# BUTSpeechFIT/DiariZen

Hardware: AMD Instinct MI355X
Metric: audio-seconds/s (RTF) for wavlm-large-s80 pipeline, 16 kHz mono (higher is better)
Workload: dtype f32 (operands split into 2 fp16 terms with exact power-of-two scaling = 22 significant bits, 3 fp16 MFMA products, fp32 accumulate: the error-corrected '3xFP16/3xTF32' scheme; kernels without an fp16 variant use the 3-term bf16 split)

## Files before the change

diarizen_amd/_lib.py:

```python
from __future__ import annotations

import ctypes as C
import os
from pathlib import Path

DZN_MAX_CONV = 8
DZN_MAX_LAYERS = 32
DZN_MAX_HEADS = 16

DZN_PREC_F32 = 0
DZN_PREC_BF16 = 1
DZN_PREC_F32_SPLIT = 2
DZN_PREC_F32_H2 = 3
DZN_PREC_F16 = 4

DZN_ACT_NONE, DZN_ACT_GELU, DZN_ACT_SWISH, DZN_ACT_RELU = 0, 1, 2, 3

DZN_F32, DZN_F64, DZN_I64 = 0, 1, 2

ERRORS = {0: "ok", -1: "invalid argument", -2: "out of memory", -3: "HIP runtime error",
          -4: "bad call order", -5: "missing state_dict key"}


class DznError(RuntimeError):
    pass


class DznConfig(C.Structure):
    _fields_ = [
        ("struct_size", C.c_int32),
        ("precision", C.c_int32),
        ("max_batch", C.c_int32),
        ("max_samples", C.c_int32),
        ("extractor_layer_norm", C.c_int32),
        ("normalize_waveform", C.c_int32),
        ("n_conv", C.c_int32),
        ("conv_ch", C.c_int32 * DZN_MAX_CONV),
        ("conv_k", C.c_int32 * DZN_MAX_CONV),
        ("conv_s", C.c_int32 * DZN_MAX_CONV),
        ("embed_dim", C.c_int32),
        ("total_heads", C.c_int32),
        ("n_layers", C.c_int32),
        ("layer_norm_first", C.c_int32),
        ("pos_conv_kernel", C.c_int32),
        ("pos_conv_groups", C.c_int32),
        ("num_buckets", C.c_int32),
        ("max_distance", C.c_int32),
        ("use_attention", C.c_int32 * DZN_MAX_LAYERS),
        ("n_heads", C.c_int32 * DZN_MAX_LAYERS),
        ("head_idx", (C.c_int32 * DZN_MAX_HEADS) * DZN_MAX_LAYERS),
        ("use_ffn", C.c_int32 * DZN_MAX_LAYERS),
        ("ffn_dim", C.c_int32 * DZN_MAX_LAYERS),
        ("attention_in", C.c_int32),
        ("ffn_hidden", C.c_int32),
        ("conf_heads", C.c_int32),
        ("conf_layers", C.c_int32),
        ("conf_kernel", C.c_int32),
        ("n_classes", C.c_int32),
        ("max_speakers_per_chunk", C.c_int32),
        ("max_speakers_per_frame", C.c_int32),
        ("has_embedding", C.c_int32),
        ("embed_out_dim", C.c_int32),
        ("num_mel_bins", C.c_int32),
        ("reserved", C.c_int32 * 16),
    ]


class DznGemmDesc(C.Structure):
    _fields_ = [
        ("A", C.c_void_p), ("W", C.c_void_p), ("W16", C.c_void_p), ("C", C.c_void_p),
        ("bias", C.c_void_p), ("R", C.c_void_p), ("WS", C.c_void_p),
        ("a_rowoff", C.c_void_p), ("c_rowoff", C.c_void_p),
        ("M", C.c_int32), ("N", C.c_int32), ("K", C.c_int32),
        ("lda", C.c_int64), ("kc", C.c_int32), ("ldk", C.c_int64), ("ldw", C.c_int32),
        ("ldc", C.c_int64), ("ldws", C.c_int64),
        ("act", C.c_int32), ("alpha", C.c_float), ("post_relu", C.c_int32),
        ("ws_w", C.c_float), ("ws_init", C.c_int32),
        ("nz", C.c_int32), ("zdiv", C.c_int32),
        ("a_z0", C.c_int64), ("a_z1", C.c_int64), ("w_z0", C.c_int64), ("w_z1", C.c_int64),
        ("c_z0", C.c_int64), ("c_z1", C.c_int64), ("b_z0", C.c_int64), ("b_z1", C.c_int64),
        ("precision", C.c_int32),
        ("alg_flops", C.c_double),
        ("a_bf16", C.c_int32), ("c_bf16", C.c_int32), ("r_bf16", C.c_int32),
        ("W3", C.c_void_p),
        ("a_split3", C.c_int32), ("a_plane", C.c_int64),
        ("ln_stats", C.c_void_p), ("ln_colsum", C.c_void_p),
        ("W2h", C.c_void_p), ("col_scale", C.c_void_p), ("a_amax", C.c_void_p), ("c_amax", C.c_void_p),
        ("amax_unit", C.c_int32),
        ("stat_partial", C.c_void_p), ("stat_final", C.c_void_p), ("stat_C", C.c_int32), ("stat_eps", C.c_float),
        ("z_count", C.c_void_p), ("z_list", C.c_void_p), ("ln_centered", C.c_int32),
        ("Wmx", C.c_void_p), ("col_scale_mx", C.c_void_p),
        ("amax_count", C.c_int32),
        ("kv_planes", C.c_void_p), ("kv_plane_stride", C.c_int64), ("kv_scale", C.c_void_p), ("kv_ld", C.c_int32),
        ("kv_col0", C.c_int32),
    ]


class DznProfEntry(C.Structure):
    _fields_ = [("name", C.c_char * 64), ("launches", C.c_int64), ("ms", C.c_double),
                ("flops", C.c_double), ("bytes", C.c_double)]


def lib_path() -> Path:
    env = os.environ.get("DZN_HIP_LIB")
    if env:
        return Path(env)
    return Path(__file__).resolve().parent / "lib" / "libdzn_hip.so"


_LIB = None


def load() -> C.CDLL:
    global _LIB
    if _LIB is not None:
        return _LIB
    p = lib_path()
    if not p.exists():
        raise DznError(
            f"{p} not found: build the HIP extension first (python -m diarizen_amd.build). "
            "diarizen_amd has no CPU fallback.")
    try:
        import torch
    except Exception:
        pass
    lib = C.CDLL(str(p))
    vp, i32, i64, f32 = C.c_void_p, C.c_int32, C.c_int64, C.c_float

    def sig(name, res, args):
        fn = getattr(lib, name)
        fn.restype = res
        fn.argtypes = args

    sig("dzn_create", i32, [C.POINTER(DznConfig), C.POINTER(vp)])
    sig("dzn_load_tensor", i32, [vp, C.c_char_p, vp, C.POINTER(i64), i32, i32])
    sig("dzn_finalize_weights", i32, [vp])
    sig("dzn_num_frames", i32, [vp, i32])
    sig("dzn_segment_forward", i32, [vp, vp, i32, i32, vp, vp, vp])
    sig("dzn_embed_forward", i32, [vp, vp, vp, i32, i32, i32, i32, vp, vp])
    sig("dzn_prepare_masks", i32, [vp, vp, i32, i32, i32, i32, i32, vp, vp, vp])
    sig("dzn_speaker_count", i32, [vp, i32, i32, i32, vp, i32, vp, vp, vp])
    sig("dzn_cluster_activations", i32, [vp, vp, i32, i32, i32, vp, i32, i32, vp, vp])
    sig("dzn_detect", i32, [vp, i32, i32, i32, vp, vp, i32, i32, f32, f32, vp, vp, vp])
    sig("dzn_debug_fetch", i32, [vp, C.c_char_p, vp, i64, C.POINTER(i64)])
    sig("dzn_embed_skip_stats", i32, [vp, C.POINTER(i64), C.POINTER(i64)])
    sig("dzn_num_ignored", i32, [vp])
    sig("dzn_workspace_bytes", i64, [vp])
    sig("dzn_last_error", C.c_char_p, [vp])
    sig("dzn_destroy", i32, [vp])
    sig("dzn_version", C.c_char_p, [])
    sig("dzn_profile_enable", i32, [i32])
    sig("dzn_profile_collect", i32, [C.POINTER(DznProfEntry), i32, C.POINTER(i32)])
    sig("dzn_profile_reserve", i32, [i32])
    sig("dzn_op_relpos_bucket", i32, [i32, i32, i32])
    sig("dzn_linkage_centroid", i32, [vp, i32, i32, vp, i32])
    sig("dzn_cdist_cosine", i32, [vp, i32, i32, vp, i32, vp, i32])
    sig("dzn_host_workspace_release", i32, [i32])
    sig("dzn_host_workspace_bytes", i64, [i32])
    sig("dzn_vbx_create", i32, [vp, vp, vp, i32, i32, i32, i32, C.POINTER(C.c_void_p)])
    sig("dzn_vbx_stats", i32, [vp, vp])
    sig("dzn_vbx_estep", i32, [vp, vp, vp, vp, C.c_double, C.POINTER(C.c_double)])
    sig("dzn_vbx_gamma", i32, [vp, vp])
    sig("dzn_vbx_destroy", i32, [vp])
    sig("dzn_op_gemm", i32, [C.POINTER(DznGemmDesc), vp])
    sig("dzn_op_split_weights", i32, [vp, i64, i32, i64, vp, vp])
    sig("dzn_op_split_weights_h2", i32, [vp, i64, i32, i64, vp, vp, vp])
    sig("dzn_op_split_weights_mx", i32, [vp, i64, i32, i64, vp, vp, vp])
    sig("dzn_op_set_gemm_mx_cfg", i32, [C.c_char_p])
    sig("dzn_checked_status", i32, [vp, i32])
    sig("dzn_flac_info", i32, [vp, C.c_size_t, vp, vp, vp, vp, vp])
    sig("dzn_flac_decode", i32, [vp, C.c_size_t, vp, i64, vp])
    sig("dzn_op_set_gemm_cfg", i32, [C.c_char_p])
    sig("dzn_op_amax", i32, [vp, i64, vp, vp])
    sig("dzn_op_split_rows", i32, [vp, vp, i64, i64, i32, vp])
    sig("dzn_op_conv3x3_c32", i32, [vp, vp, vp, vp, vp, i32, i32, i32, i32, i32, vp])
    sig("dzn_op_resblock_ws", i32, [vp, vp, vp, vp, vp, vp, vp, vp, vp, f32, f32, i32, i32, i32, i32, vp])
    sig("dzn_op_resblock32_fused", i32, [vp, vp, vp, vp, vp, vp, vp, vp, vp, f32, f32, i32, i32, i32, vp])
    sig("dzn_op_set_resblock_np", i32, [i32])
    sig("dzn_op_set_attention_noskip", i32, [i32])
    sig("dzn_op_conv3x3_c32_h2", i32, [vp, vp, vp, vp, vp, vp, vp, vp, i32, i32, i32, i32, i32, vp])
    sig("dzn_op_layernorm", i32, [vp, i64, vp, i64, vp, vp, i64, i32, i32, f32, i32, vp])
    sig("dzn_op_gate", i32, [vp, i64, vp, vp, vp, vp, i64, i32, vp])
    sig("dzn_op_row_stats", i32, [vp, i64, i64, i32, f32, vp, vp])
    sig("dzn_op_gate_stats", i32, [vp, i64, vp, vp, vp, vp, vp, vp, vp, i64, i32, f32, vp])
    sig("dzn_op_attention_h2", i32, [vp, vp, vp, vp, vp, i32, i32, i32, i32, i32, i32, f32, vp, vp])
    sig("dzn_op_set_attention_qb", i32, [i32])
    sig("dzn_op_set_attention_prefetch", i32, [i32])
    sig("dzn_op_attention_planes", i32, [vp, vp, vp, vp, vp, i32, i32, i32, i32, i32, i32, f32, vp, vp, vp, vp])
    sig("dzn_op_attention", i32, [vp, vp, vp, vp, vp, i32, i32, i32, i32, i32, i32, f32, i32, vp])
    _LIB = lib
    return lib


EXPORTED = [
    "dzn_create", "dzn_load_tensor", "dzn_finalize_weights", "dzn_num_frames",
    "dzn_segment_forward", "dzn_embed_forward", "dzn_prepare_masks", "dzn_speaker_count", "dzn_cluster_activations", "dzn_detect", "dzn_debug_fetch", "dzn_embed_skip_stats", "dzn_num_ignored",
    "dzn_workspace_bytes", "dzn_last_error", "dzn_destroy", "dzn_version", "dzn_linkage_centroid", "dzn_cdist_cosine", "dzn_host_workspace_release",
    "dzn_host_workspace_bytes",
    "dzn_flac_info", "dzn_flac_decode", "dzn_vbx_create", "dzn_vbx_stats", "dzn_vbx_estep", "dzn_vbx_gamma", "dzn_vbx_destroy",
    "dzn_op_gemm", "dzn_op_split_weights", "dzn_op_split_weights_h2", "dzn_op_split_weights_mx", "dzn_op_set_gemm_mx_cfg", "dzn_checked_status", "dzn_op_set_gemm_cfg", "dzn_op_amax", "dzn_op_conv3x3_c32", "dzn_op_conv3x3_c32_h2", "dzn_op_resblock32_fused", "dzn_op_resblock_ws", "dzn_op_set_resblock_np", "dzn_op_set_attention_noskip", "dzn_op_split_rows", "dzn_op_layernorm", "dzn_op_row_stats", "dzn_op_gate", "dzn_op_gate_stats", "dzn_op_attention", "dzn_op_attention_h2", "dzn_op_attention_planes", "dzn_op_set_attention_qb", "dzn_op_set_attention_prefetch",
    "dzn_profile_enable", "dzn_profile_collect", "dzn_profile_reserve", "dzn_op_relpos_bucket",
]


def profile_enable(on: bool) -> None:
    check(load().dzn_profile_enable(int(on)), None, "dzn_profile_enable")


def profile_reserve(n_events: int) -> None:
    check(load().dzn_profile_reserve(int(n_events)), None, "dzn_profile_reserve")


def profile_collect() -> list:
    lib = load()
    arr = (DznProfEntry * 512)()
    n = C.c_int32(0)
    check(lib.dzn_profile_collect(arr, 512, C.byref(n)), None, "dzn_profile_collect")
    return [dict(name=arr[i].name.decode(), launches=arr[i].launches, ms=arr[i].ms,
                 flops=arr[i].flops, bytes=arr[i].bytes) for i in range(min(n.value, 512))]


def check(rc: int, handle=None, what: str = "") -> None:
    if rc == 0:
        return
    msg = ERRORS.get(rc, f"error {rc}")
    try:
        detail = load().dzn_last_error(handle)
        if detail:
            msg += ": " + detail.decode(errors="replace")
    except Exception:
        pass
    if rc == -2:
        raise MemoryError(f"{what}: {msg}")
    raise DznError(f"{what}: {msg}")
```

diarizen_amd/csrc/attention.hip:

```cpp
#include "common.h"

namespace {

template <bool BIAS, typename TO>
__global__ __launch_bounds__(256) void attn_kernel(const float* __restrict__ qkv,
                                                   TO* __restrict__ out,
                                                   const float* __restrict__ gate,
                                                   const float* __restrict__ table,
                                                   const int32_t* __restrict__ head_idx, int B,
                                                   int L, int h, int Htot, int ldqkv, int ldo,
                                                   float scale) {
  extern __shared__ __attribute__((aligned(16))) float smem_f[];
  float* sK = smem_f;
  float* sV = smem_f + 64 * 64;
  float* sT = smem_f + 2 * 64 * 64;

  const int tid = threadIdx.x, lane = tid & 63, wave = tid >> 6;
  const int lr = lane & 15, lq = lane >> 4;
  const int qt = blockIdx.x, j = blockIdx.y, b = blockIdx.z;
  const int64_t rowbase = (int64_t)b * L;
  const float* Qp = qkv + j * 64;
  const float* Kp = qkv + (h + j) * 64;
  const float* Vp = qkv + (2 * h + j) * 64;

// ... 205 lines not shown
  float wa[16], wb[16];
#pragma unroll
  for (int j = 0; j < 16; ++j) {
    wa[j] = sw[sub * 16 + j];
    wb[j] = sw[64 + sub * 16 + j];
  }
  const float ba = sw[128], bb = sw[129];
  const int C = Htot * 64;
  float gm[MAXI], bt[MAXI];
#pragma unroll
  for (int i = 0; i < MAXI; ++i) {
    gm[i] = i < Htot ? gamma[lane + 64 * i] : 0.f;
    bt[i] = i < Htot ? beta[lane + 64 * i] : 0.f;
  }
  float* sr = sy[wave];
  for (int64_t row = (int64_t)blockIdx.x * 4 + wave; row < rows; row += (int64_t)gridDim.x * 4) {
    const float* xp = x + row * ldx;
    float v[MAXI];
    float sum = 0.f;
#pragma unroll
    for (int i = 0; i < MAXI; ++i) {
      v[i] = i < Htot ? xp[lane + 64 * i] : 0.f;
      sum += v[i];
    }
    const float mean = wave_sum(sum) / (float)C;
    float sq = 0.f;
#pragma unroll
    for (int i = 0; i < MAXI; ++i) {
      const float dv = i < Htot ? v[i] - mean : 0.f;
      sq += dv * dv;
    }
    const float rstd = 1.0f / sqrtf(wave_sum(sq) / (float)C + eps);
    if (lane == 0) *reinterpret_cast<float2*>(stats + 2 * row) = make_float2(mean, rstd);
    __builtin_amdgcn_wave_barrier();
#pragma unroll
    for (int i = 0; i < MAXI; ++i)
      if (i < Htot) {
        const int e = lane + 64 * i;
        sr[e + (e >> 4)] = (v[i] - mean) * rstd * gm[i] + bt[i];
      }
    __builtin_amdgcn_s_waitcnt(0xc07f);
    __builtin_amdgcn_wave_barrier();
    for (int H0 = 0; H0 < Htot; H0 += 16) {
      const int H = H0 + (lane >> 2);
      float ta = 0.f, tb = 0.f;
      if (H < Htot) {
        const int e0 = H * 64 + sub * 16;
        const float* yp = sr + e0 + (e0 >> 4);
#pragma unroll
        for (int j = 0; j < 16; ++j) {
          ta = fmaf(yp[j], wa[j], ta);
          tb = fmaf(yp[j], wb[j], tb);
        }
      }
      ta = dpp_add<0xB1, 0xF>(ta);
      ta = dpp_add<0x4E, 0xF>(ta);
      tb = dpp_add<0xB1, 0xF>(tb);
      tb = dpp_add<0x4E, 0xF>(tb);
      if (H < Htot && sub == 0) {
        const float ga = 1.0f / (1.0f + expf(-(ta + ba)));
        const float gb = 1.0f / (1.0f + expf(-(tb + bb)));
        gate[row * Htot + H] = ga * (gb * cst[H] - 1.0f) + 2.0f;
      }
    }
  }
}

}

int launch_gate_stats(const float* x, int64_t ldx, const float* gamma, const float* beta, const float* Wg,
                      const float* bg, const float* cst, float* gate, float* stats, int64_t rows, int Htot, float eps,
                      hipStream_t s) {
  if (rows <= 0) return DZN_OK;
  if (Htot < 1 || Htot > 16) return DZN_E_INVALID;
  int pid = prof_enabled() ? prof_begin(s, "gate_ln_stats", 0.0, (double)rows * Htot * 64 * 4.0) : -1;
  int64_t grid = cdiv64(rows, 4);
  grid = grid > 256 * 8 ? 256 * 8 : grid;
  hipLaunchKernelGGL(gate_stats_kernel<16>, dim3((unsigned)grid), dim3(256), 0, s, x, ldx, gamma, beta, Wg,
                     bg, cst, gate, stats, rows, Htot, eps);
  prof_end(pid, s);
  return hipGetLastError() == hipSuccess ? DZN_OK : DZN_E_HIP;
}

extern "C" int dzn_op_gate_stats(const float* x, int64_t ldx, const float* gamma, const float* beta, const float* Wg,
                                 const float* bg, const float* cst, float* gate, float* stats, int64_t rows,
                                 int32_t Htot, float eps, void* stream) {
  if (!x || !gamma || !beta || !Wg || !bg || !cst || !gate || !stats) return DZN_E_INVALID;
  return launch_gate_stats(x, ldx, gamma, beta, Wg, bg, cst, gate, stats, rows, Htot, eps,
                           reinterpret_cast<hipStream_t>(stream));
}

int launch_attention_t(const float* qkv, void* out, int out_bf16, const float* gate, const float* table,
                       const int32_t* head_idx, int B, int L, int h, int Htot, int ldqkv, int ldo,
                       float scale, hipStream_t s) {
  if (h <= 0 || B <= 0 || L <= 0) return DZN_OK;
  const bool bias = gate && table && head_idx;
  const size_t lds = (2 * 64 * 64 + (bias ? (2 * L - 1) : 0)) * sizeof(float);
  if (lds > 160 * 1024) return DZN_E_INVALID;
  dim3 grid((L + 63) / 64, h, B);
  const int pid = prof_begin(s, bias ? "attention_relpos_f32" : "attention_f32",
                             4.0 * B * h * (double)L * L * 64.0,
                             (double)B * L * h * 64.0 * 4.0 * 4.0 + (gate ? (double)B * L * Htot * 4.0 : 0.0));
#define DZN_ATT(BIASV, T)                                                                          \
  hipLaunchKernelGGL((attn_kernel<BIASV, T>), grid, dim3(256), lds, s, qkv, static_cast<T*>(out), gate, \
                     table, head_idx, B, L, h, Htot, ldqkv, ldo, scale)
  if (bias) {
    if (out_bf16) DZN_ATT(true, u16); else DZN_ATT(true, float);
  } else {
    if (out_bf16) DZN_ATT(false, u16); else DZN_ATT(false, float);
  }
#undef DZN_ATT
  prof_end(pid, s);
  return hipGetLastError() == hipSuccess ? DZN_OK : DZN_E_HIP;
}

int launch_attention(const float* qkv, float* out, const float* gate, const float* table,
                     const int32_t* head_idx, int B, int L, int h, int Htot, int ldqkv, int ldo,
                     float scale, int precision, hipStream_t s) {
  if (prec_is_split(precision))
    return launch_attention_split(qkv, out, gate, table, head_idx, B, L, h, Htot, ldqkv, ldo, scale, s);
  return launch_attention_t(qkv, out, 0, gate, table, head_idx, B, L, h, Htot, ldqkv, ldo, scale, s);
}

int launch_gate_t(const void* y, int y_bf16, int64_t ldy, const float* Wg, const float* bg,
                  const float* cst, float* gate, int64_t rows, int Htot, hipStream_t s) {
  ProfScope prof_scope_(s, "gate", 0.0, (double)rows * Htot * (64.0 + 1.0) * 4.0);
  if (rows <= 0) return DZN_OK;
  if (y_bf16)
    hipLaunchKernelGGL(gate_kernel<u16>, dim3((unsigned)cdiv64(rows, 4)), dim3(256), 0, s,
                       static_cast<const u16*>(y), ldy, Wg, bg, cst, gate, rows, Htot);
  else
    hipLaunchKernelGGL(gate_kernel<float>, dim3((unsigned)cdiv64(rows, 4)), dim3(256), 0, s,
                       static_cast<const float*>(y), ldy, Wg, bg, cst, gate, rows, Htot);
  return hipGetLastError() == hipSuccess ? DZN_OK : DZN_E_HIP;
}

int launch_gate(const float* y, int64_t ldy, const float* Wg, const float* bg, const float* cst,
                float* gate, int64_t rows, int Htot, hipStream_t s) {
  return launch_gate_t(y, 0, ldy, Wg, bg, cst, gate, rows, Htot, s);
}

extern "C" int dzn_op_attention(const float* qkv, float* out, const float* gate,
                                const float* table, const int32_t* head_idx, int32_t B, int32_t L,
                                int32_t h, int32_t Htot, int32_t ldqkv, int32_t ldo, float scale,
                                int32_t precision, void* stream) {
  if (!qkv || !out) return DZN_E_INVALID;
  return launch_attention(qkv, out, gate, table, head_idx, B, L, h, Htot, ldqkv, ldo, scale,
                          precision, reinterpret_cast<hipStream_t>(stream));
}

extern "C" int dzn_op_gate(const float* y, int64_t ldy, const float* Wg, const float* bg,
                           const float* cst, float* gate, int64_t rows, int32_t Htot,
                           void* stream) {
  return launch_gate(y, ldy, Wg, bg, cst, gate, rows, Htot, reinterpret_cast<hipStream_t>(stream));
}
```

diarizen_amd/csrc/common.h:

```cpp
#pragma once
#include <hip/hip_runtime.h>
#include <stdint.h>
#include <math.h>
#include <string.h>
#include "../../include/dzn.h"
#include "../../include/dzn_ops.h"

typedef float f32x4 __attribute__((ext_vector_type(4)));
typedef __bf16 bf16x8 __attribute__((ext_vector_type(8)));
typedef __bf16 bf16x4 __attribute__((ext_vector_type(4)));
typedef unsigned short u16;

#define DZN_WAVE 64

template <int CTRL, int ROW_MASK>
__device__ __forceinline__ float dpp_add(float v) {
  const int t = __builtin_amdgcn_update_dpp(ROW_MASK == 0xF ? __float_as_int(v) : 0, __float_as_int(v), CTRL,
                                            ROW_MASK, 0xF, false);
  return v + __int_as_float(t);
}
__device__ __forceinline__ float wave_sum(float v) {
  v = dpp_add<0xB1, 0xF>(v);
  v = dpp_add<0x4E, 0xF>(v);
  v = dpp_add<0x124, 0xF>(v);
// ... 6 lines not shown
#pragma unroll
  for (int o = 32; o > 0; o >>= 1) v = fmaxf(v, __shfl_xor(v, o, 64));
  return v;
}

__device__ __forceinline__ void track_amax_lane(float* tracker, float m) {
  if (m > 0.f) {
    const unsigned cur = __hip_atomic_load(reinterpret_cast<unsigned int*>(tracker), __ATOMIC_RELAXED, __HIP_MEMORY_SCOPE_AGENT);
    if (__float_as_uint(m) > cur) atomicMax(reinterpret_cast<unsigned int*>(tracker), __float_as_uint(m));
  }
}
__device__ __forceinline__ void track_amax(float* tracker, float wave_partial) {
  const float m = wave_max(wave_partial);
  if ((threadIdx.x & 63) == 0) track_amax_lane(tracker, m);
}

__device__ __forceinline__ float erf_as(float x) {
  const float ax = fabsf(x);
  const float t = __builtin_amdgcn_rcpf(fmaf(0.3275911f, ax, 1.0f));
  float p = fmaf(1.061405429f, t, -1.453152027f);
  p = fmaf(p, t, 1.421413741f);
  p = fmaf(p, t, -0.284496736f);
  p = fmaf(p, t, 0.254829592f);
  const float e = __builtin_amdgcn_exp2f(-1.4426950408889634f * ax * ax);
  const float y = fmaf(-p * t, e, 1.0f);
  return copysignf(y, x);
}
__device__ __forceinline__ float gelu_erf(float x) {
  return 0.5f * x * (1.0f + erf_as(x * 0.70710678118654752440f));
}
__device__ __forceinline__ float sigmoidf_(float x) { return 1.0f / (1.0f + expf(-x)); }
__device__ __forceinline__ float swishf_(float x) { return x * sigmoidf_(x); }

__device__ __forceinline__ float apply_act(float v, int act) {
  switch (act) {
    case DZN_ACT_GELU: return gelu_erf(v);
    case DZN_ACT_SWISH: return swishf_(v);
    case DZN_ACT_RELU: return fmaxf(v, 0.0f);
    default: return v;
  }
}

__device__ __forceinline__ float ld_act(const float* p, int64_t i) { return p[i]; }
__device__ __forceinline__ float ld_act(const u16* p, int64_t i) {
  return __uint_as_float(((unsigned int)p[i]) << 16);
}
__device__ __forceinline__ void st_act(float* p, int64_t i, float v) { p[i] = v; }
__device__ __forceinline__ void st_act(u16* p, int64_t i, float v) {
  __bf16 h = (__bf16)v;
  p[i] = *reinterpret_cast<u16*>(&h);
}

static inline u16 f32_to_bf16_host(float f) {
  uint32_t u;
  memcpy(&u, &f, 4);
  if ((u & 0x7fffffffu) > 0x7f800000u) return (u16)((u >> 16) | 0x40);
  uint32_t r = 0x7fffu + ((u >> 16) & 1u);
  return (u16)((u + r) >> 16);
}

static inline bool prec_is_h2(int p) { return p == DZN_PREC_F32_H2 || p == DZN_PREC_F16; }
static inline bool prec_is_split(int p) { return p == DZN_PREC_F32_SPLIT || prec_is_h2(p); }

int launch_gemm(const dzn_gemm_desc& d, hipStream_t s);
#ifdef DZN_TUNING
int launch_gemm_lowp(const dzn_gemm_desc& d, hipStream_t s);
#endif
int launch_gemm_split(const dzn_gemm_desc& d, hipStream_t s);
int launch_gemm_split_pre(const dzn_gemm_desc& d, hipStream_t s);
int launch_pad_rows_split3(const float* x, void* planes, int64_t plane_stride, int B, int L, int Lp, int pad, int D,
                           hipStream_t st, int cg = 0, int cgp = 0);
int launch_pad_rows_split2(const float* x, void* planes, int64_t plane_stride, int B, int L, int Lp, int pad, int D,
                           const float* amax, float* snapshot, hipStream_t st, int cg = 0, int cgp = 0);
int launch_split_weights(const float* W, int64_t rows, int K, int64_t ldw, void* W3, hipStream_t s);
int launch_split_weights_h2(const float* W, int64_t rows, int K, int64_t ldw, void* W2, float* col_scale, hipStream_t s);
int host_stage_stream(int device, hipStream_t* stream);
int host_state_lease(int device, size_t bytes, hipStream_t* stream, char** base);
void host_state_release(int device);
int launch_gemm_mx(const dzn_gemm_desc& d, hipStream_t s);
int launch_split_weights_mx(const float* W, int64_t rows, int K, int64_t ldw, void* Wmx, float* col_scale, hipStream_t s);
int launch_amax(const float* x, int64_t n, float* amax, hipStream_t s);
int launch_fill_u32(void* p, unsigned value, int64_t n, hipStream_t st);
int launch_stats_finalize(const float* partial, int64_t rows, int P, int C, float eps, float* stats, hipStream_t s);
int launch_layernorm(const float* x, int64_t ldx, float* y, int64_t ldy, const float* g,
                     const float* b, int64_t rows, int C, int Cpad, float eps, int gelu,
                     hipStream_t s);
int launch_layernorm_t(const void* x, int x_bf16, int64_t ldx, void* y, int y_bf16, int64_t ldy,
                       const float* g, const float* b, const float* post, int64_t rows, int C, int Cpad,
                       float eps, int gelu, hipStream_t s, float* amax = nullptr, int64_t amax_unit = 0);
int launch_cast_bf16(const float* x, void* y, int64_t n, hipStream_t s);
int launch_row_stats(const float* x, int64_t ldx, int64_t rows, int C, float eps, float* stats, hipStream_t s);
int launch_gate_stats(const float* x, int64_t ldx, const float* gamma, const float* beta, const float* Wg,
                      const float* bg, const float* cst, float* gate, float* stats, int64_t rows, int Htot, float eps,
                      hipStream_t s);
int launch_wave_stats(const float* w, int B, int N, float eps, float* stats, hipStream_t s);
int launch_gate(const float* y, int64_t ldy, const float* Wg, const float* bg, const float* cst,
                float* gate, int64_t rows, int Htot, hipStream_t s);
int launch_gate_t(const void* y, int y_bf16, int64_t ldy, const float* Wg, const float* bg,
                  const float* cst, float* gate, int64_t rows, int Htot, hipStream_t s);
int launch_attention_t(const float* qkv, void* out, int out_bf16, const float* gate, const float* table,
                       const int32_t* head_idx, int B, int L, int h, int Htot, int ldqkv, int ldo,
                       float scale, hipStream_t s);
int launch_attention_split(const float* qkv, float* out, const float* gate, const float* table,
                           const int32_t* head_idx, int B, int L, int h, int Htot, int ldqkv, int ldo,
                           float scale, hipStream_t s, const float* amax = nullptr);
int launch_attention(const float* qkv, float* out, const float* gate, const float* table,
                     const int32_t* head_idx, int B, int L, int h, int Htot, int ldqkv, int ldo,
                     float scale, int precision, hipStream_t s);
int launch_attention_planes(const float* qkv, const void* planes, int64_t plane_stride, const float* kvs, int kv_ld, float* out,
                            const float* gate, const float* table, const int32_t* head_idx, int B, int L, int h, int Htot,
                            int ldqkv, int ldo, float scale, hipStream_t s, const float* amax);

int launch_conv0(const float* wave, int B, int N, const float* stats, const float* w,
                 const float* gamma, const float* beta, int C0, int Cp, int k, int s, int T0,
                 int layer_norm, float eps, void* out, int out_bf16, hipStream_t st, const float* lnq = nullptr);
int launch_groupnorm_gelu(const float* x, void* y, int y_bf16, int B, int T, int C, int Cp, int64_t ld,
                          const float* gamma, const float* beta, float eps, float* stats, hipStream_t st, float* amax = nullptr);
int64_t gn_stats_floats(int B, int T, int C, int Cp);
int launch_pad_rows(const float* x, void* xpad, int out_bf16, int B, int L, int Lp, int pad, int D,
                    hipStream_t st);
int launch_ws_accum(const float* x, float* ws, float w, int init, int64_t n, hipStream_t st);
constexpr int WS_SUM_MAX = 40;
struct WsSumArgs {
  const float* x[WS_SUM_MAX];
  float w[WS_SUM_MAX];
  int n;
};
int launch_ws_sum(const WsSumArgs& a, float* ws, int64_t n, hipStream_t st);
int launch_col_scale(void* x, int x_bf16, int64_t rows, int C, int64_t ld, const float* scale,
                     hipStream_t st);
int launch_split_weights_h2_natural(const float* W, int64_t rows, int K, void* W2, float* col_scale, hipStream_t s);
int launch_fragment_major(const void* W2, int rows, int K, void* out, hipStream_t s);
int launch_conv01_fused(const float* wave, int B, int N, const float* wstats, const float* w0, const float* gamma0,
                        const float* beta0, const float* lnq, int C0, int T0, int T1, const void* W2h,
                        const float* col_scale, int N1p, float act_bound, float eps, float* out, hipStream_t st,
                        const float* gamma1 = nullptr, const float* beta1 = nullptr, int C1 = 0, float* amax1 = nullptr);
int launch_glu_dwconv(const float* u, int64_t ldu, const float* w, const float* bias, void* out,
                      int out_bf16, int64_t ldo, int B, int L, int A, int ks, hipStream_t st);
int launch_classify(const float* z, int64_t ldz, const float* W, const float* bias,
                    const uint8_t* mapping, int64_t rows, int A, int NC, int S, float* logp,
                    uint8_t* multilabel, hipStream_t st);
int launch_frame_prep(const float* wave, int B, int N, int T, int flen, int fshift, int Kp,
                      const float* window, float preemph, float* frames, hipStream_t st);
int launch_power(const float* spec, int64_t rows, int nb, float* pw, hipStream_t st);
int launch_window_active(const float* masks, int B, int per_window, int* flag, hipStream_t st);
int launch_compact_active(const int* flag, int B, int* count, int* list, long long* totals, hipStream_t st);
int launch_log_cmn(float* mel, int B, int T, int NB, float eps, hipStream_t st);
int launch_stem_conv(const float* fb, int B, int T, int NB, int C, const float* w, const float* bias,
                     void* img, int out_bf16, hipStream_t st, float* amax = nullptr, const int* z_count = nullptr,
                     const int* z_list = nullptr);
int launch_stats_pool(const void* img, int in_bf16, int B, int H, int W, int C, const float* masks, int S,
                      int L, float* stats, hipStream_t st, const int* active = nullptr);

int launch_conv3x3_c32_split(const float* in, const void* W3, const float* bias, const float* R, float* out, int B,
                             int Hs, int Ws, int relu, int post_relu, hipStream_t s, float* amax = nullptr,
                             const void* W2h = nullptr, const float* col_scale = nullptr, const float* amax_in = nullptr,
                             const int* z_count = nullptr, const int* z_list = nullptr);

int launch_resblock32_fused(const float* in, float* out, const void* W1, const float* cs1, const float* b1, const void* W2,
                            const float* cs2, const float* b2, const float* amax_in, float* amax_out, float l1max1,
                            float bmax1, int B, int Hs, int Ws, int np, hipStream_t s, const int* z_count = nullptr,
                            const int* z_list = nullptr);

int launch_resblock_ws(const float* in, float* out, const void* W1, const float* cs1, const float* b1, const void* W2,
                       const float* cs2, const float* b2, const float* amax_in, float* amax_out, float l1max1, float bmax1,
                       int B, int Hs, int Ws, int C, hipStream_t s, const int* z_count = nullptr, const int* z_list = nullptr,
// ... 60 lines not shown
```

diarizen_amd/csrc/engine.cpp:

```cpp
#include <algorithm>
#include <cmath>
#include <cstdio>
#include <cstdlib>
#include <map>
#include <set>
#include <stdexcept>
#include <string>
#include <vector>

#include "common.h"

#define HIPCHK(x)                                                                        \
  do {                                                                                   \
    hipError_t e_ = (x);                                                                 \
    if (e_ != hipSuccess) {                                                              \
      throw EngineError(e_ == hipErrorOutOfMemory ? DZN_E_NOMEM : DZN_E_HIP,             \
                        std::string(#x) + ": " + hipGetErrorString(e_));                 \
    }                                                                                    \
  } while (0)

namespace {

struct EngineError : std::runtime_error {
  int code;
  EngineError(int c, const std::string& m) : std::runtime_error(m), code(c) {}
};


struct HostT {
  std::vector<float> v;
  std::vector<int64_t> shape;
};

struct Lin {
  float* W = nullptr;
  u16* W16 = nullptr;
  u16* W3 = nullptr;
  float* b = nullptr;
  u16* W2h = nullptr;
  float* wsc = nullptr;
  float* csum = nullptr;
  unsigned char* Wmx = nullptr;
  float* wsc_mx = nullptr;
  int N = 0, K = 0;
  int Nt = 0, Kt = 0;
};

struct LNp {
  float* g = nullptr;
  float* b = nullptr;
  int C = 0;
};

struct EncLayer {
  bool attn = false, ffn = false;
  int h = 0, F = 0, Fp = 0;
  LNp ln1, ln2;
  Lin qkv, out, f1, f2;
  float *Wg = nullptr, *bg = nullptr, *cst = nullptr;
  int32_t* head_idx = nullptr;
};

struct ConfLayer {
  LNp ffn1_ln, ffn2_ln, mha_ln, conv_ln, out_ln;
  Lin ffn1_w1, ffn1_w2, ffn2_w1, ffn2_w2, qkv, o, pw1, pw2;
  float *dw = nullptr, *dwb = nullptr;
};

struct ResConv {
  Lin l;
  int cin = 0, cout = 0, ksz = 3, stride = 1;
  float l1max = 0.f, bmax = 0.f;
};
struct ResBlock {
  ResConv c1, c2, sc;
  bool has_sc = false;
};

std::string last_create_error;

const char* const F16_CLASSES[] = {"conv gemm", "feature projection", "pos conv", "qkv", "out_proj", "ffn1", "ffn2", "proj",
                                   "conf ffn w1", "conf ffn w2", "conf qkv", "conf out", "conf pw1", "conf pw2"};
int f16_class(const char* what) {
  for (int i = 0; i < (int)(sizeof(F16_CLASSES) / sizeof(F16_CLASSES[0])); ++i)
    if (!strcmp(what, F16_CLASSES[i])) return i;
  return -1;
}

}

struct dzn_handle {
  dzn_config cfg{};
  int device = 0;
  std::string err;
  std::map<std::string, HostT> sd;
  std::set<std::string> used;
  int ignored = 0;
  bool finalized = false;
  bool debug = false;
  std::vector<void*> allocs;
  int64_t bytes = 0;
  std::map<std::string, std::vector<float>> taps;

  int nconv = 0;
  int C[DZN_MAX_CONV]{}, Cp[DZN_MAX_CONV]{};
  int D = 0, H = 0, A = 0, Fh = 0;
  float* conv0_w = nullptr;
  float* conv0_lnq = nullptr;
  u16* conv1_W2n = nullptr;
  float* conv1_wscn = nullptr;
  LNp conv_ln[DZN_MAX_CONV];
  Lin conv[DZN_MAX_CONV];
  float* dummy_w = nullptr;
  LNp fp_ln, enc_ln;
  Lin fp, posconv;
  int pos_rowD = 0;
  int pos_cgp = 0;
  std::vector<EncLayer> layers;
  std::vector<float> rel_embed;
  std::vector<float> wsum_w;
  Lin proj;
  LNp lnorm;
  std::vector<ConfLayer> conf;
  float *cls_w = nullptr, *cls_b = nullptr;
  uint8_t* mapping = nullptr;
  int table_L = -1;
  int pos_L = -1;
  int32_t* pos_rowoff = nullptr;
  u16* xpad3 = nullptr;
  int64_t xpad3_plane = 0;
  float* table = nullptr;
  int maxT[DZN_MAX_CONV]{};
  int maxL = 0;
  float *stats = nullptr, *gn_stats = nullptr, *bufA = nullptr, *bufB = nullptr, *craw = nullptr;
  float *x = nullptr, *xpad = nullptr, *y = nullptr, *ws = nullptr, *qkv = nullptr, *ao = nullptr,
        *gate = nullptr, *mid = nullptr;
  float *hz = nullptr, *ht = nullptr, *hmid = nullptr, *hv = nullptr;
  void* kvp = nullptr;
  float* kvs = nullptr;
  int64_t kvp_rows = 0;
  int kvp_ldmax = 0;
  float* xl = nullptr;
// ... 318 lines not shown
    }
  }
  const int last = c.n_conv - 1;
  {
    const HostT& dw = need(h, P + "feature_extractor.dummy_weight");
    expect_numel(dw, h->C[last], "dummy_weight");
    h->dummy_w = upload(h, dw.v);
  }
  const int D = h->D;
  h->fp_ln = ln_from_sd(h, P + "encoder.feature_projection.layer_norm", h->C[last]);
  if (h->fold_ln)
    h->fp = linear_ln_from_sd(h, P + "encoder.feature_projection.projection",
                              P + "encoder.feature_projection.layer_norm", D, h->C[last], D, h->Cp[last]);
  else
    h->fp = linear_from_sd(h, P + "encoder.feature_projection.projection", D, h->C[last], D,
                           h->Cp[last]);
  {
    const std::string pc = P + "encoder.transformer.pos_conv_embed.conv";
    const HostT& g = need(h, pc + ".parametrizations.weight.original0");
    const HostT& v = need(h, pc + ".parametrizations.weight.original1");
    const HostT& b = need(h, pc + ".bias");
    const int K = c.pos_conv_kernel, G = c.pos_conv_groups, cg = D / G;
    expect_numel(g, K, pc + ".original0");
    expect_numel(v, (int64_t)D * cg * K, pc + ".original1");
    expect_numel(b, D, pc + ".bias");
    std::vector<double> nrm(K, 0.0);
    for (int o = 0; o < D; ++o)
      for (int ii = 0; ii < cg; ++ii)
        for (int j = 0; j < K; ++j) {
          const double t = v.v[((size_t)o * cg + ii) * K + j];
          nrm[j] += t * t;
        }
    const int cgp = prec_is_split(c.precision) ? round_up(cg, 32) : cg;
    h->pos_cgp = cgp;
    std::vector<float> wp((size_t)D * K * cgp, 0.f);
    for (int o = 0; o < D; ++o)
      for (int ii = 0; ii < cg; ++ii)
        for (int j = 0; j < K; ++j) {
          const float nj = (float)std::sqrt(nrm[j]);
          wp[((size_t)o * K + j) * cgp + ii] = g.v[j] * v.v[((size_t)o * cg + ii) * K + j] / nj;
        }
    h->posconv = make_lin(h, wp, b.v.data(), D, K * cgp, D, K * cgp);
    h->posconv.Kt = K * cg;
  }
  if (!c.layer_norm_first) h->enc_ln = ln_from_sd(h, P + "encoder.transformer.layer_norm", D);
  h->layers.resize(c.n_layers);
  int maxQ = 64, maxF = 32;
  for (int i = 0; i < c.n_layers; ++i) {
    EncLayer& L = h->layers[i];
    const std::string lp = P + "encoder.transformer.layers." + std::to_string(i);
    L.attn = c.use_attention[i] && c.n_heads[i] > 0;
    L.ffn = c.use_ffn[i] != 0;
    L.ln1 = ln_from_sd(h, lp + ".layer_norm", D);
    L.ln2 = ln_from_sd(h, lp + ".final_layer_norm", D);
    if (L.attn) {
      L.h = c.n_heads[i];
      const int hd = L.h * 64;
      maxQ = std::max(maxQ, hd);
      std::vector<float> wq((size_t)3 * hd * D), bq((size_t)3 * hd);
      const char* names[3] = {".attention.q_proj", ".attention.k_proj", ".attention.v_proj"};
      for (int t = 0; t < 3; ++t) {
        const HostT& w = need(h, lp + names[t] + ".weight");
        const HostT& b = need(h, lp + names[t] + ".bias");
        expect_numel(w, (int64_t)hd * D, lp + names[t] + ".weight");
        expect_numel(b, hd, lp + names[t] + ".bias");
        std::copy(w.v.begin(), w.v.end(), wq.begin() + (size_t)t * hd * D);
        std::copy(b.v.begin(), b.v.end(), bq.begin() + (size_t)t * hd);
      }
      if (h->fold_ln && c.layer_norm_first)
        L.qkv = make_lin_ln(h, wq, bq.data(), need(h, lp + ".layer_norm.weight").v,
                            need(h, lp + ".layer_norm.bias").v, 3 * hd, D, 3 * hd, D);
      else
        L.qkv = make_lin(h, wq, bq.data(), 3 * hd, D, 3 * hd, D);
      L.out = linear_from_sd(h, lp + ".attention.out_proj", D, hd, D, hd);
      const HostT& wg = need(h, lp + ".attention.gru_rel_pos_linear.weight");
      const HostT& bg = need(h, lp + ".attention.gru_rel_pos_linear.bias");
      const HostT& cs = need(h, lp + ".attention.gru_rel_pos_const");
      expect_numel(wg, 8 * 64, "gru_rel_pos_linear.weight");
      expect_numel(bg, 8, "gru_rel_pos_linear.bias");
      expect_numel(cs, h->H, "gru_rel_pos_const");
      L.Wg = upload(h, wg.v);
      L.bg = upload(h, bg.v);
      L.cst = upload(h, cs.v);
      std::vector<int32_t> hi(c.head_idx[i], c.head_idx[i] + L.h);
      for (int v : hi)
        if (v < 0 || v >= h->H) throw EngineError(DZN_E_INVALID, "head index out of range");
      L.head_idx = dalloc<int32_t>(h, L.h, false);
      HIPCHK(hipMemcpy(L.head_idx, hi.data(), L.h * sizeof(int32_t), hipMemcpyHostToDevice));
      if (i == 0) {
        const HostT& e = need(h, lp + ".attention.rel_attn_embed.weight");
        expect_numel(e, (int64_t)c.num_buckets * h->H, "rel_attn_embed.weight");
        h->rel_embed = e.v;
      }
    }
    if (L.ffn) {
      L.F = c.ffn_dim[i];
      L.Fp = pad32(L.F);
      maxF = std::max(maxF, L.Fp);
      if (h->fold_ln && c.layer_norm_first)
        L.f1 = linear_ln_from_sd(h, lp + ".feed_forward.intermediate_dense", lp + ".final_layer_norm", L.F, D,
                                 L.Fp, D);
      else
        L.f1 = linear_from_sd(h, lp + ".feed_forward.intermediate_dense", L.F, D, L.Fp, D);
      L.f2 = linear_from_sd(h, lp + ".feed_forward.output_dense", D, L.F, D, L.Fp);
    }
  }
  if (h->rel_embed.empty())
    throw EngineError(DZN_E_INVALID, "layer 0 must carry attention (rel_attn_embed lives there)");
  {
    const HostT& w = need(h, "weight_sum.weight");
    expect_numel(w, c.n_layers + 1, "weight_sum.weight");
    h->wsum_w = w.v;
  }
  const int A = h->A, Fh = h->Fh;
  h->proj = linear_from_sd(h, "proj", A, D, A, D);
  h->lnorm = ln_from_sd(h, "lnorm", A);
  h->conf.resize(c.conf_layers);
  for (int i = 0; i < c.conf_layers; ++i) {
    ConfLayer& L = h->conf[i];
    const std::string cp = "conformer.conformer_layer." + std::to_string(i);
    L.ffn1_ln = ln_from_sd(h, cp + ".ffn1.ln_norm", A);
    L.ffn1_w1 = h->fold_ln ? linear_ln_from_sd(h, cp + ".ffn1.w_1", cp + ".ffn1.ln_norm", Fh, A, Fh, A)
                           : linear_from_sd(h, cp + ".ffn1.w_1", Fh, A, Fh, A);
    L.ffn1_w2 = linear_from_sd(h, cp + ".ffn1.w_2", A, Fh, A, Fh);
    L.ffn2_ln = ln_from_sd(h, cp + ".ffn2.ln_norm", A);
    L.ffn2_w1 = h->fold_ln ? linear_ln_from_sd(h, cp + ".ffn2.w_1", cp + ".ffn2.ln_norm", Fh, A, Fh, A)
                           : linear_from_sd(h, cp + ".ffn2.w_1", Fh, A, Fh, A);
    L.ffn2_w2 = linear_from_sd(h, cp + ".ffn2.w_2", A, Fh, A, Fh);
    L.mha_ln = ln_from_sd(h, cp + ".mha.ln_norm", A);
    {
      std::vector<float> wq((size_t)3 * A * A), bq((size_t)3 * A);
      const char* names[3] = {".mha.mha.linearQ", ".mha.mha.linearK", ".mha.mha.linearV"};
      for (int t = 0; t < 3; ++t) {
        const HostT& w = need(h, cp + names[t] + ".weight");
        const HostT& b = need(h, cp + names[t] + ".bias");
        expect_numel(w, (int64_t)A * A, cp + names[t] + ".weight");
        expect_numel(b, A, cp + names[t] + ".bias");
        std::copy(w.v.begin(), w.v.end(), wq.begin() + (size_t)t * A * A);
        std::copy(b.v.begin(), b.v.end(), bq.begin() + (size_t)t * A);
      }
      if (h->fold_ln)
        L.qkv = make_lin_ln(h, wq, bq.data(), need(h, cp + ".mha.ln_norm.weight").v,
                            need(h, cp + ".mha.ln_norm.bias").v, 3 * A, A, 3 * A, A);
      else
        L.qkv = make_lin(h, wq, bq.data(), 3 * A, A, 3 * A, A);
    }
    L.o = linear_from_sd(h, cp + ".mha.mha.linearO", A, A, A, A);
    L.conv_ln = ln_from_sd(h, cp + ".conv.ln_norm", A);
    L.pw1 = h->fold_ln ? linear_ln_from_sd(h, cp + ".conv.pointwise_conv1", cp + ".conv.ln_norm", 2 * A, A, 2 * A, A)
                       : linear_from_sd(h, cp + ".conv.pointwise_conv1", 2 * A, A, 2 * A, A);
    L.pw2 = linear_from_sd(h, cp + ".conv.pointwise_conv2", A, A, A, A);
    {
      const int ks = c.conf_kernel;
      const HostT& w = need(h, cp + ".conv.depthwise_conv.weight");
      const HostT& b = need(h, cp + ".conv.depthwise_conv.bias");
      const HostT& g = need(h, cp + ".conv.bn_norm.weight");
      const HostT& be = need(h, cp + ".conv.bn_norm.bias");
      const HostT& rm = need(h, cp + ".conv.bn_norm.running_mean");
      const HostT& rv = need(h, cp + ".conv.bn_norm.running_var");
      expect_numel(w, (int64_t)A * ks, cp + ".conv.depthwise_conv.weight");
      std::vector<float> wf((size_t)A * ks), bf(A);
      for (int ch = 0; ch < A; ++ch) {
        const float s = g.v[ch] / std::sqrt(rv.v[ch] + 1e-5f);
        for (int j = 0; j < ks; ++j) wf[(size_t)ch * ks + j] = w.v[(size_t)ch * ks + j] * s;
        bf[ch] = (b.v[ch] - rm.v[ch]) * s + be.v[ch];
      }
// ... 467 lines not shown
  const bool fold = h->fold_ln;
  auto folded = [&](dzn_gemm_desc& d, const Lin& l) {
    d.ln_stats = h->rstat;
    d.ln_colsum = l.csum;
  };
  if (fold) {
    chk(launch_row_stats(cur, h->Cp[last], ML, h->C[last], 1e-5f, h->rstat, st), "row_stats");
    dzn_gemm_desc d = gd(h, cur, h->fp, h->x, ML, h->Cp[last], D);
    folded(d, h->fp);
    if (lnx && c.n_conv > 1) d.a_amax = am(conv_slot(cur));
    d.c_amax = am(dzn_handle::AM_X);
    gemm(d, false, false, "feature projection");
  } else {
    ln_t(cur, lp, h->Cp[last], nxt, lp, h->Cp[last], h->fp_ln, ML, h->Cp[last], 0, st);
    dzn_gemm_desc d = gd(h, nxt, h->fp, h->x, ML, h->Cp[last], D);
    d.c_amax = am(dzn_handle::AM_X);
    gemm(d, lp, false, "feature projection");
  }
  tap(h, "featproj", h->x, ML, D, D, st);

  {
    const int Kc = c.pos_conv_kernel, G = c.pos_conv_groups, cg = D / G, Lp = L + Kc;
    const bool pc16 = lp && (cg % 32 == 0);
    const int cgp = h->pos_cgp > 0 ? h->pos_cgp : cg, Dp = G * cgp;
    const bool pre3 = h->xpad3 != nullptr && (int64_t)c.max_batch * Lp * Dp < (int64_t)1 << 31;
    const bool pre2 = pre3 && h2 && h->posconv.W2h;
    if (pre2)
      chk(launch_pad_rows_split2(h->x, h->xpad3, h->xpad3_plane, B, L, Lp, Kc / 2, Dp, am(dzn_handle::AM_X),
                                 am(dzn_handle::AM_XPAD), st, cg, cgp),
          "pad_rows_split2");
    else if (pre3)
      chk(launch_pad_rows_split3(h->x, h->xpad3, h->xpad3_plane, B, L, Lp, Kc / 2, Dp, st, cg, cgp), "pad_rows_split3");
    else
      chk(launch_pad_rows(h->x, h->xpad, pc16, B, L, Lp, Kc / 2, D, st), "pad_rows");
    const int ca = pre3 ? cgp : cg, Da = pre3 ? Dp : D;
    if (!pre3 && cgp != cg) throw EngineError(DZN_E_INVALID, "padded positional-conv groups need the pre-split planes");
    const bool tabled = (int64_t)c.max_batch * Lp * Da < (int64_t)1 << 31;
    if (tabled) ensure_pos_rowoff(h, L, Lp, Da, st);
    dzn_gemm_desc d = gd(h, h->xpad, h->posconv, h->x, tabled ? ML : L, Da, D);
    d.N = cg;
    d.kc = ca;
    d.ldk = Da;
    d.act = DZN_ACT_GELU;
    d.R = h->x;
    d.a_z1 = ca;
    d.w_z1 = (int64_t)cg * h->posconv.K;
    d.c_z1 = cg;
    d.b_z1 = cg;
    if (tabled) {
      d.a_rowoff = h->pos_rowoff;
      d.nz = G;
      d.zdiv = G;
      d.alg_flops = 2.0 * (double)ML * cg * h->posconv.Kt;
    } else {
      d.nz = B * G;
      d.zdiv = G;
      d.a_z0 = (int64_t)Lp * Da;
      d.c_z0 = (int64_t)L * D;
      d.alg_flops = 2.0 * (double)L * cg * h->posconv.Kt;
    }
    if (pre3) {
      d.A = reinterpret_cast<const float*>(h->xpad3);
      d.a_split3 = pre2 ? 2 : 1;
      d.a_plane = h->xpad3_plane;
      if (pre2) d.a_amax = am(dzn_handle::AM_XPAD);
    }
    d.c_amax = am(dzn_handle::AM_X);
    gemm(d, pc16, false, "pos conv");
  }
  if (!c.layer_norm_first) ln_t(h->x, false, D, h->x, false, D, h->enc_ln, ML, D, 0, st, nullptr, am(dzn_handle::AM_X), L);
  const bool defer = h->xl != nullptr;
  float* xr = h->x;
  WsSumArgs wsum{};
  if (defer) {
    wsum.x[wsum.n] = xr;
    wsum.w[wsum.n++] = h->wsum_w[0];
  } else {
    chk(launch_ws_accum(h->x, h->ws, h->wsum_w[0], 1, ML * D, st), "ws_accum");
  }
  tap(h, "rep0", h->x, ML, D, D, st);

  static const bool stats_from_epilogue = getenv("DZN_NO_EPILOGUE_STATS") == nullptr;
  ensure_table(h, L, st);
  for (int i = 0; i < c.n_layers; ++i) {
    EncLayer& Ly = h->layers[i];
    const float wl = h->wsum_w[i + 1];
    float* const own = defer ? h->xl + (int64_t)i * ML * D : xr;
    bool have_stats = false;
    if (Ly.attn) {
      const float* yin = xr;
      bool y16 = false;
      const bool fold1 = fold && c.layer_norm_first;
      if (fold1) {
        chk(launch_gate_stats(xr, D, Ly.ln1.g, Ly.ln1.b, Ly.Wg, Ly.bg, Ly.cst, h->gate, h->rstat, ML, h->H, 1e-5f,
                              st),
            "gate_stats");
      } else if (c.layer_norm_first) {
        ln_t(xr, false, D, h->y, lp, D, Ly.ln1, ML, D, 0, st, nullptr, am(dzn_handle::AM_Y), L);
        yin = h->y;
        y16 = lp;
      } else if (lp) {
        chk(launch_cast_bf16(xr, h->y, ML * D, st), "cast");
        yin = h->y;
        y16 = true;
      }
      if (!fold1) chk(launch_gate_t(yin, y16, D, Ly.Wg, Ly.bg, Ly.cst, h->gate, ML, h->H, st), "gate");
      const int hd = Ly.h * 64;
      dzn_gemm_desc d = gd(h, yin, Ly.qkv, h->qkv, ML, D, 3 * hd);
      if (fold1) folded(d, Ly.qkv);
      d.a_amax = am(yin == xr ? dzn_handle::AM_X : dzn_handle::AM_Y);
      d.c_amax = am(dzn_handle::AM_QKV);
      const bool planes = h->kvp != nullptr && !y16 && d.W2h && d.col_scale && d.a_amax;
      const int64_t pstride = (ML + 64) * (int64_t)(2 * hd);
      if (planes) {
        d.kv_planes = h->kvp;
        d.kv_plane_stride = pstride;
        d.kv_scale = h->kvs;
        d.kv_ld = 2 * hd;
        d.kv_col0 = hd;
      }
      gemm(d, y16, false, "qkv");
      if (planes)
        chk(launch_attention_planes(h->qkv, h->kvp, pstride, h->kvs, 2 * hd, h->ao, h->gate, h->table, Ly.head_idx, B, L, Ly.h, h->H,
                                    3 * hd, hd, 0.125f, st, am(dzn_handle::AM_QKV)),
            "attention");
      else if (prec_is_split(c.precision))
        chk(launch_attention_split(h->qkv, h->ao, h->gate, h->table, Ly.head_idx, B, L, Ly.h, h->H, 3 * hd, hd,
                                   0.125f, st, am(dzn_handle::AM_QKV)),
            "attention");
      else
        chk(launch_attention_t(h->qkv, h->ao, lp, h->gate, h->table, Ly.head_idx, B, L, Ly.h, h->H, 3 * hd,
                               hd, 0.125f, st),
            "attention");
      dzn_gemm_desc o = gd(h, h->ao, Ly.out, own, ML, hd, D);
      o.R = xr;
      o.a_amax = am(dzn_handle::AM_QKV);
      o.c_amax = am(dzn_handle::AM_X);
      if (fold && c.layer_norm_first && Ly.ffn && stats_from_epilogue) {
        o.stat_partial = h->spart;
        o.stat_final = h->rstat;
        o.stat_C = D;
        o.stat_eps = 1e-5f;
        have_stats = true;
      }
      gemm(o, lp, false, "out_proj");
      xr = own;
    }
    if (c.layer_norm_first) {
      if (Ly.ffn) {
        const float* fin = h->y;
        if (fold) {
          if (!have_stats) chk(launch_row_stats(xr, D, ML, D, 1e-5f, h->rstat, st), "row_stats");
          fin = xr;
        } else {
          ln_t(xr, false, D, h->y, lp, D, Ly.ln2, ML, D, 0, st, nullptr, am(dzn_handle::AM_Y), L);
        }
        dzn_gemm_desc f1 = gd(h, fin, Ly.f1, h->mid, ML, D, Ly.Fp);
        if (fold) folded(f1, Ly.f1);
        f1.act = DZN_ACT_GELU;
        f1.a_amax = am(fin == xr ? dzn_handle::AM_X : dzn_handle::AM_Y);
        f1.c_amax = am(dzn_handle::AM_MID);
        gemm(f1, lp, lp, "ffn1");
        dzn_gemm_desc f2 = gd(h, h->mid, Ly.f2, own, ML, Ly.Fp, D);
        f2.R = xr;
        if (!defer) {
          f2.WS = h->ws;
          f2.ldws = D;
          f2.ws_w = wl;
        }
        f2.a_amax = am(dzn_handle::AM_MID);
        f2.c_amax = am(dzn_handle::AM_X);
        gemm(f2, lp, false, "ffn2");
        xr = own;
      } else if (!defer) {
        chk(launch_ws_accum(xr, h->ws, wl, 0, ML * D, st), "ws_accum");
      }
      if (defer) {
        wsum.x[wsum.n] = xr;
        wsum.w[wsum.n++] = wl;
      }
    } else {
      ln_t(xr, false, D, xr, false, D, Ly.ln1, ML, D, 0, st, nullptr, am(dzn_handle::AM_X), L);
      if (Ly.ffn) {
        const float* fin = xr;
        if (lp) {
          chk(launch_cast_bf16(xr, h->y, ML * D, st), "cast");
          fin = h->y;
        }
        dzn_gemm_desc f1 = gd(h, fin, Ly.f1, h->mid, ML, D, Ly.Fp);
        f1.act = DZN_ACT_GELU;
        f1.a_amax = am(dzn_handle::AM_X);
        f1.c_amax = am(dzn_handle::AM_MID);
        gemm(f1, lp, lp, "ffn1");
        dzn_gemm_desc f2 = gd(h, h->mid, Ly.f2, xr, ML, Ly.Fp, D);
        f2.R = xr;
        f2.a_amax = am(dzn_handle::AM_MID);
        f2.c_amax = am(dzn_handle::AM_X);
        gemm(f2, lp, false, "ffn2");
      }
      ln_t(xr, false, D, xr, false, D, Ly.ln2, ML, D, 0, st, nullptr, am(dzn_handle::AM_X), L);
      chk(launch_ws_accum(xr, h->ws, wl, 0, ML * D, st), "ws_accum");
    }
    if (h->debug) {
      const std::string nm = "layer" + std::to_string(i);
      tap(h, nm.c_str(), xr, ML, D, D, st);
    }
  }
  if (defer) chk(launch_ws_sum(wsum, h->ws, ML * D, st), "ws_sum");
  tap(h, "wsum", h->ws, ML, D, D, st);

  {
    const float* pin = h->ws;
    if (lp) {
      chk(launch_cast_bf16(h->ws, h->y, ML * D, st), "cast");
      pin = h->y;
    }
    dzn_gemm_desc d = gd(h, pin, h->proj, h->hz, ML, D, A);
    gemm(d, lp, false, "proj");
    ln_t(h->hz, false, A, h->hz, false, A, h->lnorm, ML, A, 0, st, nullptr, am(dzn_handle::AM_HZ), L);
  }
  tap(h, "head_in", h->hz, ML, A, A, st);
  for (int i = 0; i < c.conf_layers; ++i) {
    ConfLayer& Cl = h->conf[i];
    auto half_ffn = [&](const LNp& ln, const Lin& w1, const Lin& w2) {
      const float* in = h->ht;
      if (fold) {
        chk(launch_row_stats(h->hz, A, ML, A, 1e-5f, h->rstat, st), "row_stats");
        in = h->hz;
      } else {
        ln_t(h->hz, false, A, h->ht, lp, A, ln, ML, A, 0, st);
      }
      dzn_gemm_desc a = gd(h, in, w1, h->hmid, ML, A, Fh);
      if (fold) folded(a, w1);
      a.act = DZN_ACT_SWISH;
      if (in == h->hz) a.a_amax = am(dzn_handle::AM_HZ);
      a.c_amax = am(dzn_handle::AM_HMID);
      gemm(a, lp, lp, "conf ffn w1");
      dzn_gemm_desc b = gd(h, h->hmid, w2, h->hz, ML, Fh, A);
      b.alpha = 0.5f;
      b.R = h->hz;
      b.a_amax = am(dzn_handle::AM_HMID);
      b.c_amax = am(dzn_handle::AM_HZ);
      gemm(b, lp, false, "conf ffn w2");
    };
    half_ffn(Cl.ffn1_ln, Cl.ffn1_w1, Cl.ffn1_w2);
    if (fold) chk(launch_row_stats(h->hz, A, ML, A, 1e-5f, h->rstat, st), "row_stats");
    else ln_t(h->hz, false, A, h->ht, lp, A, Cl.mha_ln, ML, A, 0, st);
    {
      dzn_gemm_desc q = gd(h, fold ? h->hz : h->ht, Cl.qkv, h->hmid, ML, A, 3 * A);
      if (fold) {
        folded(q, Cl.qkv);
        q.a_amax = am(dzn_handle::AM_HZ);
      }
      q.c_amax = am(dzn_handle::AM_HMID);
// ... 477 lines not shown
```

diarizen_amd/csrc/gemm.hip:

```cpp
#include <cstdio>
#include <cstdlib>

#include "common.h"
#include "gemm_epilogue.h"

namespace {

template <bool LOWP>
struct Frag {
  using type = f32x4;
};
template <>
struct Frag<true> {
  using type = bf16x8;
};

__device__ __forceinline__ uint4 pack_bf16x8(const float4& a, const float4& b) {
  bf16x8 v;
  v[0] = (__bf16)a.x; v[1] = (__bf16)a.y; v[2] = (__bf16)a.z; v[3] = (__bf16)a.w;
  v[4] = (__bf16)b.x; v[5] = (__bf16)b.y; v[6] = (__bf16)b.z; v[7] = (__bf16)b.w;
  return *reinterpret_cast<uint4*>(&v);
}

template <int BM, int BN, int WGM, int WGN, bool LOWP>
// ... 284 lines not shown
    __syncthreads();
    if (more) read_frags(buf ^ 1, 0, a0, b0);
    __builtin_amdgcn_sched_barrier(0);
    mma(a1, b1);
    __builtin_amdgcn_sched_barrier(0);
  }
  gemm_epilogue<BM, BN, TM, TN, MI, NI>(d, acc, tm, tn, wm, wn, lr, lq, cz, bz, z0);
}

template <int BM, int BN, int WGM, int WGN, bool LOWP>
int launch_cfg(const dzn_gemm_desc& d, hipStream_t s) {
  const int tilesM = (d.M + BM - 1) / BM, tilesN = (d.N + BN - 1) / BN;
  static const int lds_pad = getenv("DZN_GEMM_LDS_PAD") ? atoi(getenv("DZN_GEMM_LDS_PAD")) : 0;
  const size_t lds = 2 * (BM + BN) * 128 + lds_pad;
  auto kern = gemm_kernel<BM, BN, WGM, WGN, LOWP>;
  static unsigned long long attr_mask = 0;
  if (first_use_on_device(attr_mask)) {
    (void)hipFuncSetAttribute(reinterpret_cast<const void*>(kern),
                        hipFuncAttributeMaxDynamicSharedMemorySize, 160 * 1024);
    if constexpr (!LOWP)
      (void)hipFuncSetAttribute(reinterpret_cast<const void*>(gemm_glds_kernel<BM, BN, WGM, WGN>),
                                hipFuncAttributeMaxDynamicSharedMemorySize, 160 * 1024);
  }
  static const bool no_glds = getenv("DZN_NO_GLDS") != nullptr;
  const bool use_glds = !LOWP && !no_glds && (d.K % 32 == 0) && (d.kc % 32 == 0);
  dim3 grid(tilesM * tilesN, d.nz > 0 ? d.nz : 1, 1);
  int pid = -1;
  if (prof_enabled()) {
    char cls[64];
    static const bool by_shape = getenv("DZN_PROFILE_SHAPES") != nullptr;
    if (by_shape)
      snprintf(cls, sizeof(cls), "gemm_%s_%dx%d M%d N%d K%d z%d", LOWP ? "bf16" : "f32", BM, BN, d.M, d.N,
               d.K, d.nz);
    else
      snprintf(cls, sizeof(cls), "gemm_%s_%dx%d", LOWP ? "bf16" : "f32", BM, BN);
    const double fl = d.alg_flops > 0 ? d.alg_flops * d.nz : 2.0 * d.M * d.N * d.K * d.nz;
    pid = prof_begin(s, cls, fl, gemm_alg_bytes(d, LOWP ? 2 : 4));
  }
  if constexpr (!LOWP) {
    if (use_glds)
      hipLaunchKernelGGL((gemm_glds_kernel<BM, BN, WGM, WGN>), grid, dim3(256), lds, s, d);
    else
      hipLaunchKernelGGL(kern, grid, dim3(256), lds, s, d);
  } else {
    hipLaunchKernelGGL(kern, grid, dim3(256), lds, s, d);
  }
  prof_end(pid, s);
  if (hipGetLastError() != hipSuccess) return DZN_E_HIP;
  if (d.stat_partial && d.stat_final)
    return launch_stats_finalize(d.stat_partial, d.M, ((d.N + BN - 1) / BN) * WGN, d.stat_C, d.stat_eps, d.stat_final, s);
  return DZN_OK;
}

template <bool LOWP>
int launch_prec(const dzn_gemm_desc& d, hipStream_t s) {
  static const char* force = getenv("DZN_GEMM_CFG");
  if (force) {
    if (!strcmp(force, "128x32")) return launch_cfg<128, 32, 4, 1, LOWP>(d, s);
    if (!strcmp(force, "256x32")) return launch_cfg<256, 32, 4, 1, LOWP>(d, s);
    if (!strcmp(force, "256x64")) return launch_cfg<256, 64, 4, 1, LOWP>(d, s);
    if (!strcmp(force, "128x64")) return launch_cfg<128, 64, 2, 2, LOWP>(d, s);
    if (!strcmp(force, "64x64")) return launch_cfg<64, 64, 2, 2, LOWP>(d, s);
    if (!strcmp(force, "128x128")) return launch_cfg<128, 128, 2, 2, LOWP>(d, s);
  }
  if (d.N <= 32) return launch_cfg<256, 32, 4, 1, LOWP>(d, s);
  if (d.N <= 64) return launch_cfg<128, 64, 2, 2, LOWP>(d, s);
  if (d.K <= 512 && (d.N % 64) == 0) return launch_cfg<128, 64, 2, 2, LOWP>(d, s);
  const int cand[4] = {192, 160, 128, 96};
  int best = 128, best_cols = 1 << 30;
  for (int c : cand) {
    const int cols = (d.N + c - 1) / c * c;
    if (cols < best_cols) { best_cols = cols; best = c; }
  }
  switch (best) {
    case 192: return launch_cfg<128, 192, 2, 2, LOWP>(d, s);
    case 160: return launch_cfg<128, 160, 2, 2, LOWP>(d, s);
    case 96: return launch_cfg<128, 96, 2, 2, LOWP>(d, s);
    default: return launch_cfg<128, 128, 2, 2, LOWP>(d, s);
  }
}

}

int launch_gemm(const dzn_gemm_desc& din, hipStream_t s) {
  dzn_gemm_desc d = din;
  if (d.M <= 0 || d.N <= 0) return DZN_OK;
  if (d.K <= 0 || (d.K & 7)) return DZN_E_INVALID;
  if (d.kc <= 0) { d.kc = d.K; d.ldk = 0; }
  if (d.kc & 7) return DZN_E_INVALID;
  if (d.zdiv <= 0) d.zdiv = 1;
  if (d.nz <= 0) d.nz = 1;
  if (d.alpha == 0.f) d.alpha = 1.f;
  if (d.precision == DZN_PREC_BF16) {
    if (!d.W16) return DZN_E_INVALID;
#ifdef DZN_TUNING
    if (d.a_bf16) return launch_gemm_lowp(d, s);
#else
    if (d.a_bf16) return DZN_E_INVALID;
#endif
    if (d.c_bf16 || d.r_bf16) return DZN_E_INVALID;
    return launch_prec<true>(d, s);
  }
  if (!d.W) return DZN_E_INVALID;
  if (d.kv_planes) {
    const bool ok = d.kv_scale && d.precision == DZN_PREC_F32_H2 && d.W3 && d.W2h && d.col_scale && d.a_amax && !(d.K & 31) &&
                    !(d.kc & 31) && d.ldw == d.K && !d.a_split3 && d.nz == 1 && !d.c_rowoff && d.kv_col0 >= 0 &&
                    d.kv_col0 < d.N && !(d.kv_col0 & 63) && !(d.N & 63) && d.kv_ld == d.N - d.kv_col0 &&
                    !(d.kv_plane_stride & 3) && d.N > 32 && !getenv("DZN_GEMM_CFG") && !getenv("DZN_NO_H2");
    if (!ok) return DZN_E_INVALID;
  }
  if (d.ln_centered && !(d.precision == DZN_PREC_F16 && d.W3 && !(d.K & 31) && !(d.kc & 31) && d.ldw == d.K && !d.a_split3))
    return DZN_E_INVALID;
  if (d.a_split3) return prec_is_split(d.precision) ? launch_gemm_split_pre(d, s) : DZN_E_INVALID;
  if (prec_is_split(d.precision) && d.W3 && !(d.K & 31) && !(d.kc & 31) && d.ldw == d.K)
    return launch_gemm_split(d, s);
  return launch_prec<false>(d, s);
}

extern "C" int dzn_op_gemm(const dzn_gemm_desc* d, void* stream) {
  if (!d || !d->A || !d->C) return DZN_E_INVALID;
  return launch_gemm(*d, reinterpret_cast<hipStream_t>(stream));
}
```

diarizen_amd/csrc/gemm_epilogue.h:

```cpp
#pragma once
#include <type_traits>

#include "common.h"
#include "split.h"

namespace {

template <int BM, int BN, int TM, int TN, int MI, int NI, int RS = 16, int CS = 16>
__device__ __forceinline__ void gemm_epilogue_general(const dzn_gemm_desc& d, f32x4 (&acc)[MI][NI], int tm, int tn,
                                              int wm, int wn, int lr, int lq, int64_t cz, int64_t bz, int z0 = 0,
                                              const float* row_inv = nullptr, const float* col_scale = nullptr) {
  const float* __restrict__ bias = d.bias ? d.bias + bz : nullptr;
  const bool vec = (((int64_t)d.N | d.ldc | d.ldws | cz | bz) & 3) == 0;
  float amax = 0.f, amax_hi = 0.f;
  const int wrow0 = tm * BM + wm * TM;
  const bool two_unit = d.c_amax && d.amax_unit >= TM;
  const int unit0 = two_unit ? (wrow0 < d.M ? wrow0 : d.M - 1) / d.amax_unit : 0;
  const int boundary = two_unit ? (unit0 + 1) * d.amax_unit : 0;
#pragma unroll
  for (int i = 0; i < MI; ++i) {
    const int m = tm * BM + wm * TM + i * RS + lr;
    if (m >= d.M) continue;
    const int64_t crow = cz + (d.c_rowoff ? (int64_t)d.c_rowoff[m] : (int64_t)m * d.ldc);
    const float acc_scale = row_inv ? row_inv[i] : 1.f;
// ... 37 lines not shown
        *reinterpret_cast<float4*>(d.C + crow + n0) = make_float4(v[0], v[1], v[2], v[3]);
        amax_row = fmaxf(fmaxf(amax_row, fmaxf(fabsf(v[0]), fabsf(v[1]))), fmaxf(fabsf(v[2]), fabsf(v[3])));
        st_s += (v[0] + v[1]) + (v[2] + v[3]);
        st_q = fmaf(v[0], v[0], fmaf(v[1], v[1], fmaf(v[2], v[2], fmaf(v[3], v[3], st_q))));
        if (d.WS) {
          float4* w = reinterpret_cast<float4*>(d.WS + (int64_t)m * d.ldws + n0);
          float4 a = d.ws_init ? make_float4(0.f, 0.f, 0.f, 0.f) : *w;
          a.x += d.ws_w * v[0]; a.y += d.ws_w * v[1]; a.z += d.ws_w * v[2]; a.w += d.ws_w * v[3];
          *w = a;
        }
      } else {
#pragma unroll
        for (int e = 0; e < 4; ++e) {
          const int n = n0 + e;
          if (n >= d.N) continue;
          float x = v[e];
          if (col_scale) x *= acc_scale * col_scale[n];
          if (d.ln_stats) x = ln_rs * (x - ln_mu * d.ln_colsum[n]);
          if (bias) x += bias[n];
          x = apply_act(x, d.act) * d.alpha;
          if (d.R) x += d.R[crow + n];
          if (d.post_relu) x = fmaxf(x, 0.f);
          d.C[crow + n] = x;
          amax_row = fmaxf(amax_row, fabsf(x));
          st_s += x;
          st_q = fmaf(x, x, st_q);
          if (d.WS) {
            float* w = d.WS + (int64_t)m * d.ldws + n;
            *w = d.ws_init ? d.ws_w * x : (*w + d.ws_w * x);
          }
        }
      }
    }
    if (d.stat_partial) {
      float s1 = st_s, q1 = st_q;
      if constexpr (RS == 16) {
        s1 += __shfl_xor(s1, 16, 64);
        q1 += __shfl_xor(q1, 16, 64);
      }
      s1 += __shfl_xor(s1, 32, 64);
      q1 += __shfl_xor(q1, 32, 64);
      if (lq == 0) {
        const int P = ((d.N + BN - 1) / BN) * (BN / TN);
        reinterpret_cast<float2*>(d.stat_partial)[(int64_t)m * P + tn * (BN / TN) + wn] = make_float2(s1, q1);
      }
    }
    if (d.c_amax) {
      if (two_unit) {
        if (m < boundary) amax = fmaxf(amax, amax_row);
        else amax_hi = fmaxf(amax_hi, amax_row);
      } else if (d.amax_unit > 0) {
        float r = amax_row;
        if constexpr (RS == 16) r = fmaxf(r, __shfl_xor(r, 16, 64));
        r = fmaxf(r, __shfl_xor(r, 32, 64));
        if (lq == 0) track_amax_lane(d.c_amax + m / d.amax_unit, r);
      } else {
        amax = fmaxf(amax, amax_row);
      }
    }
  }
  if (two_unit) {
    track_amax(d.c_amax + unit0, amax);
    if (wrow0 + TM > boundary && boundary < d.M) track_amax(d.c_amax + unit0 + 1, amax_hi);
  } else if (d.c_amax && d.amax_unit <= 0) {
    track_amax(d.c_amax + z0, amax);
  }
}

constexpr int epi_chunk(int ni, int cap) {
  int best = 1;
  for (int c = 1; c <= cap; ++c)
    if (ni % c == 0) best = c;
  return best;
}

template <int ACT>
__device__ __forceinline__ float apply_act_c(float v) {
  if constexpr (ACT == DZN_ACT_GELU) return gelu_erf(v);
  else if constexpr (ACT == DZN_ACT_SWISH) return swishf_(v);
  else if constexpr (ACT == DZN_ACT_RELU) return fmaxf(v, 0.0f);
  else return v;
}

template <int BM, int BN, int TM, int TN, int MI, int NI, bool LDSCOLS = false, int RS = 16, int CS = 16>
__device__ __forceinline__ void gemm_epilogue(const dzn_gemm_desc& d, f32x4 (&acc)[MI][NI], int tm, int tn,
                                              int wm, int wn, int lr, int lq, int64_t cz, int64_t bz, int z0 = 0,
                                              const float* row_inv = nullptr, const float* col_scale = nullptr,
                                              float* lds_cols = nullptr, const f32x4 (*rpre)[NI] = nullptr) {
  const bool vec = (((int64_t)d.N | d.ldc | d.ldws | cz | bz) & 3) == 0 && d.N >= 4;
  if (!vec) {
    gemm_epilogue_general<BM, BN, TM, TN, MI, NI, RS, CS>(d, acc, tm, tn, wm, wn, lr, lq, cz, bz, z0, row_inv, col_scale);
    return;
  }
  const bool ring = d.R && !rpre;
  constexpr int JCMAX = MI * NI > 16 ? 4 : 8;
  constexpr int JC = epi_chunk(NI, JCMAX);
  static_assert(NI % JC == 0, "column chunks tile the wavefront tile");
  constexpr int NJC = NI / JC, NB = MI * NJC;
  constexpr bool REGCOLS = !LDSCOLS && NI <= 4;
  const float* __restrict__ bias = d.bias ? d.bias + bz : nullptr;
  const int ncol0 = tn * BN + wn * TN + lq * 4;
  auto nok_ = [&](const int j) { return ncol0 + j * CS < d.N; };
  auto nc_ = [&](const int j) {
    const int n0 = ncol0 + j * CS;
    return n0 < d.N ? n0 : d.N - 4;
  };
  int64_t crow[MI];
  bool mok[MI];
  int mcl[MI];
#pragma unroll
  for (int i = 0; i < MI; ++i) {
    const int m = tm * BM + wm * TM + i * RS + lr;
    mok[i] = m < d.M;
    mcl[i] = mok[i] ? m : d.M - 1;
    crow[i] = cz + (d.c_rowoff ? (int64_t)d.c_rowoff[mcl[i]] : (int64_t)mcl[i] * d.ldc);
  }
  float4 r4[2][JC];
  auto issue_r = [&](const int b, const int slot) {
    const int i = b / NJC, jc = b % NJC;
#pragma unroll
    for (int jj = 0; jj < JC; ++jj) r4[slot][jj] = *reinterpret_cast<const float4*>(d.R + crow[i] + nc_(jc * JC + jj));
  };
  if (ring) issue_r(0, 0);
  float ln_mu[MI], ln_rs[MI];
#pragma unroll
  for (int i = 0; i < MI; ++i) {
    ln_mu[i] = 0.f;
    ln_rs[i] = 1.f;
  }
  if (d.ln_stats) {
#pragma unroll
    for (int i = 0; i < MI; ++i) {
      const float2 st = *reinterpret_cast<const float2*>(d.ln_stats + 2 * (int64_t)mcl[i]);
      ln_mu[i] = d.ln_centered ? 0.f : st.x;
      ln_rs[i] = st.y;
    }
  }
  float4 cs4[REGCOLS ? NI : 1], lc4[REGCOLS ? NI : 1], b4[REGCOLS ? NI : 1];
  if constexpr (REGCOLS) {
#pragma unroll
    for (int j = 0; j < NI; ++j) {
      cs4[j] = make_float4(1.f, 1.f, 1.f, 1.f);
      lc4[j] = b4[j] = make_float4(0.f, 0.f, 0.f, 0.f);
    }
    if (col_scale) {
#pragma unroll
      for (int j = 0; j < NI; ++j) cs4[j] = *reinterpret_cast<const float4*>(col_scale + nc_(j));
    }
    if (d.ln_stats) {
#pragma unroll
      for (int j = 0; j < NI; ++j) lc4[j] = *reinterpret_cast<const float4*>(d.ln_colsum + nc_(j));
    }
    if (bias) {
#pragma unroll
      for (int j = 0; j < NI; ++j) b4[j] = *reinterpret_cast<const float4*>(bias + nc_(j));
    }
  } else if constexpr (LDSCOLS) {
    const int lane = lq * RS + lr;
    if (lane < TN / 4) {
      int n = tn * BN + wn * TN + 4 * lane;
      n = n < d.N ? n : d.N - 4;
      float4 c = make_float4(1.f, 1.f, 1.f, 1.f), l = make_float4(0.f, 0.f, 0.f, 0.f), bb = l;
      if (col_scale) c = *reinterpret_cast<const float4*>(col_scale + n);
      if (d.ln_stats) l = *reinterpret_cast<const float4*>(d.ln_colsum + n);
      if (bias) bb = *reinterpret_cast<const float4*>(bias + n);
      *reinterpret_cast<float4*>(lds_cols + 4 * lane) = c;
      *reinterpret_cast<float4*>(lds_cols + TN + 4 * lane) = l;
      *reinterpret_cast<float4*>(lds_cols + 2 * TN + 4 * lane) = bb;
    }
    __builtin_amdgcn_fence(__ATOMIC_RELEASE, "wavefront");
  }
  auto cols = [&](const int j, float4& c, float4& l, float4& bb) {
    if constexpr (REGCOLS) {
      c = cs4[j]; l = lc4[j]; bb = b4[j];
    } else if constexpr (LDSCOLS) {
      const float* p = lds_cols + j * CS + lq * 4;
      c = *reinterpret_cast<const float4*>(p);
      l = *reinterpret_cast<const float4*>(p + TN);
      bb = *reinterpret_cast<const float4*>(p + 2 * TN);
    } else {
      c = col_scale ? *reinterpret_cast<const float4*>(col_scale + nc_(j)) : make_float4(1.f, 1.f, 1.f, 1.f);
      l = d.ln_stats ? *reinterpret_cast<const float4*>(d.ln_colsum + nc_(j)) : make_float4(0.f, 0.f, 0.f, 0.f);
      bb = bias ? *reinterpret_cast<const float4*>(bias + nc_(j)) : make_float4(0.f, 0.f, 0.f, 0.f);
    }
  };
  float amax_row[MI], st_s[MI], st_q[MI];
#pragma unroll
  for (int i = 0; i < MI; ++i) amax_row[i] = st_s[i] = st_q[i] = 0.f;

  auto run = [&](auto actc) {
    constexpr int ACT = decltype(actc)::value;
#pragma unroll
    for (int b = 0; b < NB; ++b) {
      const int i = b / NJC, jc = b % NJC;
      if (ring && b + 1 < NB) issue_r(b + 1, (b + 1) & 1);
      const float acc_scale = (col_scale && row_inv) ? row_inv[i] : 1.f;
#pragma unroll
      for (int jj = 0; jj < JC; ++jj) {
        const int j = jc * JC + jj;
        float4 c4, l4, bb4;
        cols(j, c4, l4, bb4);
        f32x4 v = acc[i][j];
        if (col_scale) {
          v[0] *= acc_scale * c4.x; v[1] *= acc_scale * c4.y; v[2] *= acc_scale * c4.z; v[3] *= acc_scale * c4.w;
        }
        if (d.ln_stats) {
          v[0] = ln_rs[i] * (v[0] - ln_mu[i] * l4.x); v[1] = ln_rs[i] * (v[1] - ln_mu[i] * l4.y);
          v[2] = ln_rs[i] * (v[2] - ln_mu[i] * l4.z); v[3] = ln_rs[i] * (v[3] - ln_mu[i] * l4.w);
        }
        if (bias) { v[0] += bb4.x; v[1] += bb4.y; v[2] += bb4.z; v[3] += bb4.w; }
#pragma unroll
        for (int e = 0; e < 4; ++e) v[e] = apply_act_c<ACT>(v[e]) * d.alpha;
        if (rpre) {
          const f32x4 r = rpre[i][j];
          v[0] += r[0]; v[1] += r[1]; v[2] += r[2]; v[3] += r[3];
        } else if (d.R) {
          const float4 r = r4[b & 1][jj];
          v[0] += r.x; v[1] += r.y; v[2] += r.z; v[3] += r.w;
        }
        if (d.post_relu) {
#pragma unroll
          for (int e = 0; e < 4; ++e) v[e] = fmaxf(v[e], 0.f);
        }
        acc[i][j] = v;
        if (nok_(j)) {
          amax_row[i] = fmaxf(fmaxf(amax_row[i], fmaxf(fabsf(v[0]), fabsf(v[1]))), fmaxf(fabsf(v[2]), fabsf(v[3])));
          st_s[i] += (v[0] + v[1]) + (v[2] + v[3]);
          st_q[i] = fmaf(v[0], v[0], fmaf(v[1], v[1], fmaf(v[2], v[2], fmaf(v[3], v[3], st_q[i]))));
        }
        __builtin_amdgcn_sched_barrier(0x00E0 | 0x0200);
      }
      if constexpr (JC % 4 == 0 && RS == 16 && CS == 16) {
        if (d.kv_planes) {
#pragma unroll
          for (int g4 = 0; g4 < JC / 4; ++g4) {
            const int jg = jc * JC + g4 * 4;
            const int nslot = tn * BN + wn * TN + jg * CS;
            if (nslot >= d.kv_col0 && nslot < d.N) {
              float am = 0.f;
#pragma unroll
              for (int q = 0; q < 4; ++q)
                am = fmaxf(fmaxf(am, fmaxf(fabsf(acc[i][jg + q][0]), fabsf(acc[i][jg + q][1]))),
                           fmaxf(fabsf(acc[i][jg + q][2]), fabsf(acc[i][jg + q][3])));
              am = fmaxf(am, __shfl_xor(am, 16, 64));
              am = fmaxf(am, __shfl_xor(am, 32, 64));
              float ks, kinv;
              h2_scale(am, ks, kinv);
              uint16_t* p0 = reinterpret_cast<uint16_t*>(d.kv_planes) + (int64_t)mcl[i] * d.kv_ld + (nslot - d.kv_col0) + lq * 4;
              uint16_t* p1 = p0 + d.kv_plane_stride;
#pragma unroll
              for (int q = 0; q < 4; ++q) {
                f32x2 x0, x1;
                x0[0] = acc[i][jg + q][0] * ks; x0[1] = acc[i][jg + q][1] * ks;
                x1[0] = acc[i][jg + q][2] * ks; x1[1] = acc[i][jg + q][3] * ks;
                const f16x2 h0 = __builtin_convertvector(x0, f16x2), h1 = __builtin_convertvector(x1, f16x2);
                const f32x2 f0 = __builtin_convertvector(h0, f32x2), f1 = __builtin_convertvector(h1, f32x2);
                f32x2 r0, r1;
                r0[0] = x0[0] - f0[0]; r0[1] = x0[1] - f0[1]; r1[0] = x1[0] - f1[0]; r1[1] = x1[1] - f1[1];
                const f16x2 l0 = __builtin_convertvector(r0, f16x2), l1 = __builtin_convertvector(r1, f16x2);
                if (mok[i]) {
                  *reinterpret_cast<uint2*>(p0 + q * CS) = make_uint2(__builtin_bit_cast(unsigned, h0), __builtin_bit_cast(unsigned, h1));
                  *reinterpret_cast<uint2*>(p1 + q * CS) = make_uint2(__builtin_bit_cast(unsigned, l0), __builtin_bit_cast(unsigned, l1));
                }
              }
              if (lq == 0 && mok[i]) d.kv_scale[(int64_t)mcl[i] * (d.kv_ld >> 6) + ((nslot - d.kv_col0) >> 6)] = kinv;
            }
          }
        }
      }
#pragma unroll
      for (int jj = 0; jj < JC; ++jj) {
        const int j = jc * JC + jj;
        bool plain = true;
        if constexpr (JC % 4 == 0 && RS == 16 && CS == 16)
          plain = !(d.kv_planes && tn * BN + wn * TN + (j & ~3) * CS >= d.kv_col0);
        if (plain && mok[i] && nok_(j))
          *reinterpret_cast<float4*>(d.C + crow[i] + nc_(j)) = make_float4(acc[i][j][0], acc[i][j][1], acc[i][j][2], acc[i][j][3]);
      }
    }
  };
  switch (d.act) {
    case DZN_ACT_GELU: run(std::integral_constant<int, DZN_ACT_GELU>{}); break;
    case DZN_ACT_SWISH: run(std::integral_constant<int, DZN_ACT_SWISH>{}); break;
    case DZN_ACT_RELU: run(std::integral_constant<int, DZN_ACT_RELU>{}); break;
    default: run(std::integral_constant<int, DZN_ACT_NONE>{}); break;
  }
  if (d.WS) {
    float4 w4[2][JC];
    auto issue_w = [&](const int b, const int slot) {
      const int i = b / NJC, jc = b % NJC;
      const float* wrow = d.WS + (int64_t)mcl[i] * d.ldws;
#pragma unroll
      for (int jj = 0; jj < JC; ++jj) w4[slot][jj] = *reinterpret_cast<const float4*>(wrow + nc_(jc * JC + jj));
    };
#pragma unroll
    for (int s = 0; s < 2; ++s)
#pragma unroll
      for (int jj = 0; jj < JC; ++jj) w4[s][jj] = make_float4(0.f, 0.f, 0.f, 0.f);
    if (!d.ws_init) issue_w(0, 0);
#pragma unroll
    for (int b = 0; b < NB; ++b) {
      const int i = b / NJC, jc = b % NJC;
      if (!d.ws_init && b + 1 < NB) issue_w(b + 1, (b + 1) & 1);
      float* wrow = d.WS + (int64_t)mcl[i] * d.ldws;
#pragma unroll
      for (int jj = 0; jj < JC; ++jj) {
        const int j = jc * JC + jj;
        const float4 w = w4[b & 1][jj];
        if (mok[i] && nok_(j))
          *reinterpret_cast<float4*>(wrow + nc_(j)) =
              make_float4(w.x + d.ws_w * acc[i][j][0], w.y + d.ws_w * acc[i][j][1], w.z + d.ws_w * acc[i][j][2],
                          w.w + d.ws_w * acc[i][j][3]);
      }
    }
  }
  float amax = 0.f, amax_hi = 0.f;
  const int wrow0 = tm * BM + wm * TM;
  const bool two_unit = d.c_amax && d.amax_unit >= TM;
  const int unit0 = two_unit ? (wrow0 < d.M ? wrow0 : d.M - 1) / d.amax_unit : 0;
  const int boundary = two_unit ? (unit0 + 1) * d.amax_unit : 0;
#pragma unroll
  for (int i = 0; i < MI; ++i) {
    const int m = tm * BM + wm * TM + i * RS + lr;
    if (!mok[i]) continue;
    if (d.stat_partial) {
      float s1 = st_s[i], q1 = st_q[i];
      if constexpr (RS == 16) {
        s1 += __shfl_xor(s1, 16, 64);
        q1 += __shfl_xor(q1, 16, 64);
      }
      s1 += __shfl_xor(s1, 32, 64);
      q1 += __shfl_xor(q1, 32, 64);
      if (lq == 0) {
        const int P = ((d.N + BN - 1) / BN) * (BN / TN);
        reinterpret_cast<float2*>(d.stat_partial)[(int64_t)m * P + tn * (BN / TN) + wn] = make_float2(s1, q1);
      }
    }
    if (d.c_amax) {
      if (two_unit) {
        if (m < boundary) amax = fmaxf(amax, amax_row[i]);
        else amax_hi = fmaxf(amax_hi, amax_row[i]);
      } else if (d.amax_unit > 0) {
        float r = amax_row[i];
        if constexpr (RS == 16) r = fmaxf(r, __shfl_xor(r, 16, 64));
        r = fmaxf(r, __shfl_xor(r, 32, 64));
        if (lq == 0) track_amax_lane(d.c_amax + m / d.amax_unit, r);
      } else {
        amax = fmaxf(amax, amax_row[i]);
      }
    }
  }
  if (two_unit) {
// ... 30 lines not shown
```

diarizen_amd/csrc/gemm_split.hip:

```cpp
#include <cmath>
#include <cstdio>
#include <cstdlib>
#include <type_traits>

#include "checked.h"
#include "common.h"
#include "gemm_epilogue.h"
#include "split.h"

DZN_CHECKED_TU(gemm_split)

namespace {

__device__ __forceinline__ int wswz(int row) { return (0x78 >> (2 * ((row >> 2) & 3))) & 3; }

template <int N>
__device__ __forceinline__ void wait_vm_lgkm0() {
  static_assert(N >= 0 && N < 64, "vmcnt range");
  __builtin_amdgcn_s_waitcnt((N & 0xF) | ((N >> 4) << 14) | (0x7 << 4));
}

template <int BM, int BN, int WGM, int WGN, int S, int NP, int OCC = 1, int ABL = 0, bool RPF = false>
__global__ __launch_bounds__(WGM * WGN * 64, OCC) void gemm_split_kernel(const dzn_gemm_desc d, const int ngroups) {
  constexpr int NW = WGM * WGN;
  constexpr int BK = 32;
  constexpr int TM = BM / WGM, TN = BN / WGN;
  constexpr int MI = TM / 16, NI = TN / 16, MH = MI / 2;
  constexpr int RB = NW * 1024;
  constexpr int ACH = BM * 128 / RB;
  constexpr int WROWS = NW * 16;
  constexpr int WR = (BN + WROWS - 1) / WROWS;
  constexpr int SP = NP == 3 ? 3 : 2;
  constexpr int ABYTES = BM * 128, WPLANE = BN * 64, BUF = ABYTES + NP * WPLANE;
  constexpr int LPT = ACH + NP * WR;
  constexpr bool WPART = BN % WROWS != 0;
  static_assert(BM * 128 % RB == 0, "A tile must be whole rounds");
  static_assert(MI % 2 == 0, "two row halves per wavefront tile");
  static_assert(S >= 2 && (S - 1) * LPT < 64, "vmcnt range");
  extern __shared__ __attribute__((aligned(16))) unsigned char smem[];

  const int tid = threadIdx.x, lane = tid & 63;
  const int wave = __builtin_amdgcn_readfirstlane(tid >> 6);
  const int wm = wave / WGN, wn = wave % WGN;
  const int tilesN = (d.N + BN - 1) / BN;
  int t;
  {
    const int nwg = gridDim.x, bid = blockIdx.x;
    const int q = nwg >> 3, r = nwg & 7, xcd = bid & 7, idx = bid >> 3;
    t = (xcd < r ? xcd * (q + 1) : r * (q + 1) + (xcd - r) * q) + idx;
  }
  int tm, tn;
  if (ngroups <= 1) {
    tm = t / tilesN;
    tn = t % tilesN;
  } else {
    const int tilesM_ = (int)gridDim.x / tilesN;
    const int base = tilesN / ngroups, rem = tilesN % ngroups;
    int g = 0, cg = base + (rem > 0), cs = 0, r = t;
    while (r >= tilesM_ * cg) {
      r -= tilesM_ * cg;
      cs += cg;
      ++g;
      cg = base + (g < rem);
    }
    tm = r / cg;
    tn = cs + r - tm * cg;
  }
  const int z = blockIdx.y;
  int z0 = z / d.zdiv;
  const int z1 = z - z0 * d.zdiv;
  if (d.z_list) {
    if (z0 >= d.z_count[0]) return;
    z0 = d.z_list[z0];
  }
  const float* __restrict__ A = d.A + z0 * d.a_z0 + z1 * d.a_z1;
  const u16* __restrict__ W3 =
      reinterpret_cast<const u16*>(NP == 3 ? d.W3 : d.W2h) + SP * (z0 * d.w_z0 + z1 * d.w_z1);
  float a_scale[MI], row_inv[MI];
#pragma unroll
  for (int i = 0; i < MI; ++i) a_scale[i] = row_inv[i] = 1.f;
  if constexpr (NP <= 2) {
#pragma unroll
    for (int i = 0; i < MI; ++i) {
      int m = tm * BM + wm * TM + i * 16 + (lane & 15);
      m = m < d.M ? m : d.M - 1;
      const int unit = d.amax_unit > 0 ? m / d.amax_unit : z0;
      DZN_CHECK(d.amax_count <= 0 || (unit >= 0 && unit < d.amax_count), 0x101, unit);
      h2_scale(d.a_amax[unit], a_scale[i], row_inv[i]);
    }
  }
  float a_mean[MI];
#pragma unroll
  for (int i = 0; i < MI; ++i) a_mean[i] = 0.f;
  if constexpr (NP == 1) {
    if (d.ln_centered && d.ln_stats) {
#pragma unroll
      for (int i = 0; i < MI; ++i) {
        int m = tm * BM + wm * TM + i * 16 + (lane & 15);
        m = m < d.M ? m : d.M - 1;
        a_mean[i] = d.ln_stats[2 * (int64_t)m];
        a_scale[i] *= 0.5f;
        row_inv[i] *= 2.f;
      }
    }
  }
// ... 111 lines not shown
    } else {
#pragma unroll
      for (int j = 0; j < NI; ++j) acc[i][j] = mfma_np<NP>(wf[j][0], af[0], acc[i][j]);
    }
  };
  auto split = [&](const f32x4 (&a)[2], u32x4 (&af)[NP], float sc, float mu = 0.f) {
    if constexpr (ABL == 1) {
#pragma unroll
      for (int p = 0; p < NP; ++p) af[p] = __builtin_bit_cast(u32x4, a[p & 1]);
    } else if constexpr (NP == 3) {
      bf16x8 h_, m_, l_;
      split8(a[0], a[1], h_, m_, l_);
      af[0] = __builtin_bit_cast(u32x4, h_);
      af[1] = __builtin_bit_cast(u32x4, m_);
      af[2] = __builtin_bit_cast(u32x4, l_);
    } else if constexpr (NP == 2) {
      split8_h2(a[0], a[1], sc, af[0], af[1]);
    } else {
      cvt8_h1(a[0] - mu, a[1] - mu, sc, af[0]);
    }
  };

  const int nk = d.K / BK;
#pragma unroll
  for (int s = 0; s < S; ++s)
    if (s < nk) issue(s);
  auto wait_tiles = [&](auto tiles) {
    constexpr int T = decltype(tiles)::value;
    if (wfull) wait_vm_lgkm0<T * LPT>();
    else wait_vm_lgkm0<T * (LPT - NP)>();
  };
  if (nk >= S) wait_tiles(std::integral_constant<int, S - 1>{});
  else wait_vm_lgkm0<0>();
  __builtin_amdgcn_s_barrier();
  u32x4 wfa[NI][NP], wfb[NI][NP];
  f32x4 ar[MI][2];
  read_w(0, wfa);
  read_a(0, ar);
  if constexpr (ABL == 5) read_w(0, wfb);
  int stage = 0;

  auto step = [&](int kt, const u32x4 (&wc)[NI][NP], u32x4 (&wn_)[NI][NP]) {
    const bool more = kt + 1 < nk;
#pragma unroll
    for (int i = 0; i < MH; ++i) {
      u32x4 af[NP];
      split(ar[i], af, a_scale[i], a_mean[i]);
      mma(i, wc, af);
    }
    u32x4 af2[MI - MH][NP];
#pragma unroll
    for (int i = MH; i < MI; ++i) split(ar[i], af2[i - MH], a_scale[i], a_mean[i]);
    const int nstage = stage + 1 == S ? 0 : stage + 1;
    __builtin_amdgcn_sched_barrier(0);
    if (more) {
      if (kt + S <= nk) wait_tiles(std::integral_constant<int, S - 2>{});
      else wait_vm_lgkm0<0>();
      if constexpr (ABL != 4) __builtin_amdgcn_s_barrier();
      if constexpr (ABL != 3)
        if (kt + S < nk) issue(stage);
      if constexpr (ABL != 5) {
        read_w(nstage, wn_);
        read_a(nstage, ar);
      }
    }
    __builtin_amdgcn_sched_barrier(0);
#pragma unroll
    for (int i = MH; i < MI; ++i) mma(i, wc, af2[i - MH]);
    stage = nstage;
  };
  for (int kt = 0; kt < nk; kt += 2) {
    step(kt, wfa, wfb);
    if (kt + 1 < nk) step(kt + 1, wfb, wfa);
  }
  if constexpr (true) {
    __syncthreads();
    if constexpr (RPF) {
      if (use_rpre) {
        gemm_epilogue<BM, BN, TM, TN, MI, NI, true>(d, acc, tm, tn, wm, wn, lr, lq, cz, bz, z0, row_inv, NP <= 2 ? d.col_scale : nullptr,
                                                    reinterpret_cast<float*>(smem) + wave * 3 * TN, rpre);
        return;
      }
    }
    gemm_epilogue<BM, BN, TM, TN, MI, NI, true>(d, acc, tm, tn, wm, wn, lr, lq, cz, bz, z0, row_inv, NP <= 2 ? d.col_scale : nullptr,
                                                reinterpret_cast<float*>(smem) + wave * 3 * TN);
  } else {
    gemm_epilogue<BM, BN, TM, TN, MI, NI>(d, acc, tm, tn, wm, wn, lr, lq, cz, bz, z0, row_inv, NP <= 2 ? d.col_scale : nullptr);
  }
}

#ifdef DZN_TUNING
typedef float f32x16 __attribute__((ext_vector_type(16)));

template <int BM, int BN, int WGM, int WGN, int S, int NP, int OCC = 1, int PRIO = 0>
__global__ __launch_bounds__(WGM * WGN * 64, OCC) void gemm_split32_kernel(const dzn_gemm_desc d) {
  static_assert(NP == 1 || NP == 2, "fp16 forms only");
  constexpr int NW = WGM * WGN;
  constexpr int BK = 32;
  constexpr int TM = BM / WGM, TN = BN / WGN;
  constexpr int MI = TM / 32, NJ = TN / 32;
  constexpr int RB = NW * 1024;
  constexpr int ACH = BM * 128 / RB;
  constexpr int WROWS = NW * 16;
  constexpr int WR = (BN + WROWS - 1) / WROWS;
  constexpr int ABYTES = BM * 128, WPLANE = BN * 64, BUF = ABYTES + NP * WPLANE;
  constexpr int LPT = ACH + NP * WR;
  constexpr bool WPART = BN % WROWS != 0;
  static_assert(BM * 128 % RB == 0 && TM % 32 == 0 && TN % 32 == 0, "tile geometry");
  static_assert(S >= 2 && (S - 1) * LPT < 64, "vmcnt range");
  extern __shared__ __attribute__((aligned(16))) unsigned char smem[];

  const int tid = threadIdx.x, lane = tid & 63;
  const int wave = __builtin_amdgcn_readfirstlane(tid >> 6);
  const int wm = wave / WGN, wn = wave % WGN;
  const int tilesN = (d.N + BN - 1) / BN;
  int t;
  {
    const int nwg = gridDim.x, bid = blockIdx.x;
    const int q = nwg >> 3, r = nwg & 7, xcd = bid & 7, idx = bid >> 3;
    t = (xcd < r ? xcd * (q + 1) : r * (q + 1) + (xcd - r) * q) + idx;
  }
  const int tm = t / tilesN, tn = t % tilesN;
  const int z = blockIdx.y;
  int z0 = z / d.zdiv;
  const int z1 = z - z0 * d.zdiv;
  if (d.z_list) {
    if (z0 >= d.z_count[0]) return;
    z0 = d.z_list[z0];
  }
  const float* __restrict__ A = d.A + z0 * d.a_z0 + z1 * d.a_z1;
  const u16* __restrict__ W2 = reinterpret_cast<const u16*>(d.W2h) + 2 * (z0 * d.w_z0 + z1 * d.w_z1);
  const int l31 = lane & 31, lh = lane >> 5;
  float a_scale[MI], row_inv[MI];
#pragma unroll
  for (int i = 0; i < MI; ++i) {
    int m = tm * BM + wm * TM + i * 32 + l31;
    m = m < d.M ? m : d.M - 1;
    h2_scale(d.a_amax[d.amax_unit > 0 ? m / d.amax_unit : z0], a_scale[i], row_inv[i]);
  }
  const int64_t cz = z0 * d.c_z0 + z1 * d.c_z1;
  const int64_t bz = z0 * d.b_z0 + z1 * d.b_z1;

  const int r0 = tid >> 3;
  const int csw = (tid & 7) ^ ((r0 >> 1) & 7);
  const float* aptr[ACH];
#pragma unroll
  for (int i = 0; i < ACH; ++i) {
    int m = tm * BM + r0 + 8 * NW * i;
    m = m < d.M ? m : d.M - 1;
    aptr[i] = A + (d.a_rowoff ? (int64_t)d.a_rowoff[m] : (int64_t)m * d.lda) + csw * 4;
  }
  const bool wfull = !WPART || (WR - 1) * WROWS + wave * 16 < BN;
  const int wr0 = wave * 16 + (lane >> 2);
  const int wsw = (lane & 3) ^ wswz(wr0);
  const u16* wptr[WR];
#pragma unroll
  for (int i = 0; i < WR; ++i) {
    int n = tn * BN + wr0 + WROWS * i;
    n = n < d.N ? n : d.N - 1;
    wptr[i] = W2 + (int64_t)n * 2 * d.ldw + wsw * 8;
  }
  int ik = 0, irem = 0;
  int64_t ikoff = 0;
  auto issue = [&](int stage) {
    unsigned char* sA = smem + stage * BUF + wave * 1024;
    unsigned char* sW = smem + stage * BUF + ABYTES + wave * 1024;
#pragma unroll
    for (int i = 0; i < ACH; ++i)
// ... 63 lines not shown
  };
  auto mma = [&](int i, int kh, const u32x4 (&wf)[NJ][2][NP], const u32x4 (&af)[NP]) {
    if constexpr (PRIO) __builtin_amdgcn_s_setprio(1);
    if constexpr (NP == 2) {
      constexpr int PW[3] = {1, 0, 0}, PA[3] = {0, 1, 0};
#pragma unroll
      for (int t = 0; t < 3; ++t)
#pragma unroll
        for (int j = 0; j < NJ; ++j) acc[i][j] = mfma32(wf[j][kh][PW[t]], af[PA[t]], acc[i][j]);
    } else {
#pragma unroll
      for (int j = 0; j < NJ; ++j) acc[i][j] = mfma32(wf[j][kh][0], af[0], acc[i][j]);
    }
    if constexpr (PRIO) __builtin_amdgcn_s_setprio(0);
  };
  auto split = [&](const f32x4 (&a)[2], u32x4 (&af)[NP], float sc) {
    if constexpr (NP == 2) split8_h2(a[0], a[1], sc, af[0], af[1]);
    else cvt8_h1(a[0], a[1], sc, af[0]);
  };

  const int nk = d.K / BK;
#pragma unroll
  for (int s = 0; s < S; ++s)
    if (s < nk) issue(s);
  auto wait_tiles = [&](auto tiles) {
    constexpr int T = decltype(tiles)::value;
    if (wfull) wait_vm_lgkm0<T * LPT>();
    else wait_vm_lgkm0<T * (LPT - NP)>();
  };
  if (nk >= S) wait_tiles(std::integral_constant<int, S - 1>{});
  else wait_vm_lgkm0<0>();
  __builtin_amdgcn_s_barrier();
  u32x4 wfa[NJ][2][NP], wfb[NJ][2][NP];
  f32x4 ar[MI][2][2];
  read_w(0, wfa);
  read_a(0, ar);
  int stage = 0;

  auto step = [&](int kt, const u32x4 (&wc)[NJ][2][NP], u32x4 (&wn_)[NJ][2][NP]) {
    const bool more = kt + 1 < nk;
#pragma unroll
    for (int i = 0; i < MI; ++i) {
      u32x4 af[NP];
      split(ar[i][0], af, a_scale[i]);
      mma(i, 0, wc, af);
    }
    u32x4 af2[MI][NP];
#pragma unroll
    for (int i = 0; i < MI; ++i) split(ar[i][1], af2[i], a_scale[i]);
    const int nstage = stage + 1 == S ? 0 : stage + 1;
    __builtin_amdgcn_sched_barrier(0);
    if (more) {
      if (kt + S <= nk) wait_tiles(std::integral_constant<int, S - 2>{});
      else wait_vm_lgkm0<0>();
      __builtin_amdgcn_s_barrier();
      if (kt + S < nk) issue(stage);
      read_w(nstage, wn_);
      read_a(nstage, ar);
    }
    __builtin_amdgcn_sched_barrier(0);
#pragma unroll
    for (int i = 0; i < MI; ++i) mma(i, 1, wc, af2[i]);
    stage = nstage;
  };
  for (int kt = 0; kt < nk; kt += 2) {
    step(kt, wfa, wfb);
    if (kt + 1 < nk) step(kt + 1, wfb, wfa);
  }
  __syncthreads();
  f32x4 accv[MI][4 * NJ];
#pragma unroll
  for (int i = 0; i < MI; ++i)
#pragma unroll
    for (int j = 0; j < NJ; ++j)
#pragma unroll
      for (int g = 0; g < 4; ++g)
#pragma unroll
        for (int e = 0; e < 4; ++e) accv[i][4 * j + g][e] = acc[i][j][4 * g + e];
  gemm_epilogue<BM, BN, TM, TN, MI, 4 * NJ, true, 32, 8>(d, accv, tm, tn, wm, wn, l31, lh, cz, bz, z0, row_inv, d.col_scale,
                                                       reinterpret_cast<float*>(smem) + wave * 3 * TN);
}

template <int BM, int BN, int WGM, int WGN, int S, int NP, int OCC = 1, int PRIO = 0>
int launch_split32_cfg(const dzn_gemm_desc& d, hipStream_t s) {
  const int tilesM = (d.M + BM - 1) / BM, tilesN = (d.N + BN - 1) / BN;
  const size_t lds = (size_t)S * (BM * 128 + NP * BN * 64);
  auto kern = gemm_split32_kernel<BM, BN, WGM, WGN, S, NP, OCC, PRIO>;
  static unsigned long long attr_mask = 0;
  if (first_use_on_device(attr_mask))
    (void)hipFuncSetAttribute(reinterpret_cast<const void*>(kern), hipFuncAttributeMaxDynamicSharedMemorySize, 160 * 1024);
  dim3 grid(tilesM * tilesN, d.nz > 0 ? d.nz : 1, 1);
  int pid = -1;
  if (prof_enabled()) {
    char cls[64];
    static const bool by_shape = getenv("DZN_PROFILE_SHAPES") != nullptr;
    if (by_shape)
      snprintf(cls, sizeof(cls), "gemm_%s_%dx%d M%d N%d K%d z%d", NP == 2 ? "f32h" : "f16", BM, BN, d.M, d.N, d.K, d.nz);
    else
      snprintf(cls, sizeof(cls), "gemm_%s_%dx%d", NP == 2 ? "f32h" : "f16", BM, BN);
    const double fl = d.alg_flops > 0 ? d.alg_flops * d.nz : 2.0 * d.M * d.N * d.K * d.nz;
    pid = prof_begin(s, cls, fl, gemm_alg_bytes(d, NP * 2));
  }
  hipLaunchKernelGGL(kern, grid, dim3(WGM * WGN * 64), lds, s, d);
  prof_end(pid, s);
  if (hipGetLastError() != hipSuccess) return DZN_E_HIP;
  if (d.stat_partial && d.stat_final)
    return launch_stats_finalize(d.stat_partial, d.M, tilesN * WGN, d.stat_C, d.stat_eps, d.stat_final, s);
  return DZN_OK;
}

#endif

int choose_column_groups(const dzn_gemm_desc& d, int tilesM, int tilesN, int BM, int NP) {
  static const char* env = getenv("DZN_GEMM_NGROUPS");
  static const bool automatic = env && !strcmp(env, "auto");
  static const int forced = env && !automatic ? atoi(env) : 0;
  if (tilesN < 2 || d.w_z0 || d.w_z1 || (!automatic && forced <= 1)) return 1;
  if (forced > 0) return forced < tilesN ? (forced > 8 ? 8 : forced) : tilesN > 8 ? 8 : tilesN;
  if ((d.nz > 1) || (int64_t)tilesM * tilesN < 1024) return 1;
  const double W = (double)d.N * d.K * 2.0 * NP;
  const double a_cols = d.a_rowoff ? (double)d.kc : (d.lda > 0 && d.lda < d.K ? (double)d.lda : (double)d.K);
  const double A = (double)d.M * a_cols * 4.0;
  auto miss = [](double bytes) {
    static const double mb[] = {0.5, 1.0, 2.0, 4.0, 8.0, 12.0}, f[] = {0.02, 0.055, 0.12, 0.27, 0.69, 1.0};
    const double x = bytes / (1024.0 * 1024.0);
    if (x <= mb[0]) return f[0] * x / mb[0];
    for (int i = 1; i < 6; ++i)
      if (x <= mb[i]) return f[i - 1] + (f[i] - f[i - 1]) * (log2(x) - log2(mb[i - 1])) / (log2(mb[i]) - log2(mb[i - 1]));
    return 1.0;
  };
  int best = 1;
  const double r1 = A + tilesM * W * miss(W);
  double rbest = r1;
  for (int G = 2; G <= 8 && G <= tilesN; G *= 2) {
    const double r = G * A + tilesM * W * miss(W / G);
    if (r < rbest) { rbest = r; best = G; }
  }
  (void)BM;
  return rbest < 0.95 * r1 ? best : 1;
}

template <int BM, int BN, int WGM, int WGN, int S, int NP, int OCC = 1, int ABL = 0, bool RPF = false>
int launch_split_cfg(const dzn_gemm_desc& d, hipStream_t s) {
  const int tilesM = (d.M + BM - 1) / BM, tilesN = (d.N + BN - 1) / BN;
  const size_t lds = (size_t)S * (BM * 128 + NP * BN * 64);
  auto kern = gemm_split_kernel<BM, BN, WGM, WGN, S, NP, OCC, ABL, RPF>;
  static unsigned long long attr_mask = 0;
  if (first_use_on_device(attr_mask)) {
    (void)hipFuncSetAttribute(reinterpret_cast<const void*>(kern), hipFuncAttributeMaxDynamicSharedMemorySize,
                              160 * 1024);
  }
  dim3 grid(tilesM * tilesN, d.nz > 0 ? d.nz : 1, 1);
  int pid = -1;
  if (prof_enabled()) {
    char cls[64];
    static const bool by_shape = getenv("DZN_PROFILE_SHAPES") != nullptr;
    if (by_shape)
      snprintf(cls, sizeof(cls), "gemm_%s_%dx%d M%d N%d K%d z%d", NP == 3 ? "f32s" : NP == 2 ? "f32h" : "f16", BM, BN, d.M,
               d.N, d.K, d.nz);
    else
      snprintf(cls, sizeof(cls), "gemm_%s_%dx%d%s", NP == 3 ? "f32s" : NP == 2 ? "f32h" : "f16", BM, BN, RPF ? "_rpf" : "");
    const double fl = d.alg_flops > 0 ? d.alg_flops * d.nz : 2.0 * d.M * d.N * d.K * d.nz;
    pid = prof_begin(s, cls, fl, gemm_alg_bytes(d, NP * 2));
  }
  hipLaunchKernelGGL(kern, grid, dim3(WGM * WGN * 64), lds, s, d, choose_column_groups(d, tilesM, tilesN, BM, NP));
  prof_end(pid, s);
  if (hipGetLastError() != hipSuccess) return DZN_E_HIP;
  if (d.stat_partial && d.stat_final)
    return launch_stats_finalize(d.stat_partial, d.M, tilesN * WGN, d.stat_C, d.stat_eps, d.stat_final, s);
  return DZN_OK;
}

__global__ __launch_bounds__(256) void split_weights_kernel(const float* __restrict__ W, int64_t rows, int K,
                                                            int64_t ldw, u16* __restrict__ W3) {
  const int64_t n = rows * K;
  for (int64_t i = (int64_t)blockIdx.x * 256 + threadIdx.x; i < n; i += (int64_t)gridDim.x * 256) {
    const int64_t r = i / K;
    const int k = (int)(i - r * K);
    const float x = W[r * ldw + k];
    const __bf16 h = (__bf16)x;
    const float r1 = x - (float)h;
    const __bf16 m = (__bf16)r1;
    const float r2 = r1 - (float)m;
    const __bf16 l = (__bf16)r2;
    const int kk = k & 31;
    const int pos = 8 * ((kk & 15) >> 2) + (kk & 3) + 4 * (kk >> 4);
    u16* o = W3 + r * 3 * K + (int64_t)(k >> 5) * 96 + pos;
    o[0] = *reinterpret_cast<const u16*>(&h);
    o[32] = *reinterpret_cast<const u16*>(&m);
    o[64] = *reinterpret_cast<const u16*>(&l);
  }
}

char g_force_buf[32] = {0};
bool g_force_init = false;
const char* g_force_cfg() {
  if (!g_force_init) {
    const char* e = getenv("DZN_GEMM_CFG");
    if (e) snprintf(g_force_buf, sizeof(g_force_buf), "%s", e);
    g_force_init = true;
  }
  return g_force_buf[0] ? g_force_buf : nullptr;
}

template <int NP>
int launch_gemm_split_np(const dzn_gemm_desc& d, hipStream_t s) {
  const char* force = g_force_cfg();
  if (force) {
    if (!strcmp(force, "128x64")) return launch_split_cfg<128, 64, 4, 1, 2, NP, NP <= 2 ? 3 : 2>(d, s);
    if (!strcmp(force, "128x80")) return launch_split_cfg<128, 80, 4, 1, 2, NP, 2>(d, s);
    if (!strcmp(force, "128x32")) return launch_split_cfg<128, 32, 4, 1, 2, NP>(d, s);
    if constexpr (NP == 3) {
      if (!strcmp(force, "128x128")) return launch_split_cfg<128, 128, 2, 2, 2, NP, 2>(d, s);
    } else {
      if (!strcmp(force, "128x128w4")) return launch_split_cfg<128, 128, 4, 1, 2, NP, 2>(d, s);
    }
    if constexpr (NP == 1) {
      if (!strcmp(force, "256x128w8s3")) return launch_split_cfg<256, 128, 8, 1, 3, NP, 2>(d, s);
    }
#ifdef DZN_TUNING
    if constexpr (NP <= 2) {
      if (!strcmp(force, "m32_128x128")) return launch_split32_cfg<128, 128, 4, 1, 2, NP, 2>(d, s);
      if (!strcmp(force, "m32_128x64")) return launch_split32_cfg<128, 64, 4, 1, 2, NP, 3>(d, s);
    }
    if (!strcmp(force, "256x128")) return launch_split_cfg<256, 128, 4, 2, 2, NP>(d, s);
    if constexpr (NP != 3) {
      if (!strcmp(force, "128x128")) return launch_split_cfg<128, 128, 2, 2, 2, NP>(d, s);
    }
    if constexpr (NP <= 2) {
      if (!strcmp(force, "m32_128x128p")) return launch_split32_cfg<128, 128, 4, 1, 2, NP, 2, 1>(d, s);
      if (!strcmp(force, "m32_128x128w22")) return launch_split32_cfg<128, 128, 2, 2, 2, NP, 2>(d, s);
      if (!strcmp(force, "m32_256x128")) return launch_split32_cfg<256, 128, 4, 2, 2, NP, 1>(d, s);
      if (!strcmp(force, "m32_256x128w8")) return launch_split32_cfg<256, 128, 8, 1, 2, NP, 1>(d, s);
      if (!strcmp(force, "m32_128x64p")) return launch_split32_cfg<128, 64, 4, 1, 2, NP, 3, 1>(d, s);
      if (!strcmp(force, "256x128s3")) return launch_split_cfg<256, 128, 4, 2, 3, NP>(d, s);
      if (!strcmp(force, "256x128w8s3")) return launch_split_cfg<256, 128, 8, 1, 3, NP, 2>(d, s);
      if (!strcmp(force, "128x64s3")) return launch_split_cfg<128, 64, 4, 1, 3, NP>(d, s);
      if (!strcmp(force, "256x64s3")) return launch_split_cfg<256, 64, 8, 1, 3, NP>(d, s);
      if (!strcmp(force, "abl1")) return launch_split_cfg<128, 128, 4, 1, 2, NP, 2, 1>(d, s);
      if (!strcmp(force, "abl2")) return launch_split_cfg<128, 128, 4, 1, 2, NP, 2, 2>(d, s);
      if (!strcmp(force, "abl3")) return launch_split_cfg<128, 128, 4, 1, 2, NP, 2, 3>(d, s);
      if (!strcmp(force, "abl4")) return launch_split_cfg<128, 128, 4, 1, 2, NP, 2, 4>(d, s);
      if (!strcmp(force, "abl5")) return launch_split_cfg<128, 128, 4, 1, 2, NP, 2, 5>(d, s);
    }
#endif
  }
#ifdef DZN_TUNING
  static const int m32 = getenv("DZN_GEMM_M32") ? atoi(getenv("DZN_GEMM_M32")) : 0;
#else
  constexpr int m32 = 0;
// ... 103 lines not shown
```

diarizen_amd/csrc/norm.hip:

```cpp
#include <cstdint>
#include <initializer_list>
#include <type_traits>

#include "common.h"

namespace {

template <int MAXI, typename TI, typename TO>
__global__ __launch_bounds__(256) void layernorm_kernel(const TI* __restrict__ x, int64_t ldx,
                                                        TO* __restrict__ y, int64_t ldy,
                                                        const float* __restrict__ gamma,
                                                        const float* __restrict__ beta,
                                                        const float* __restrict__ post, int64_t rows,
                                                        int C, int Cpad, float eps, int gelu,
                                                        float* __restrict__ amax_out, int64_t amax_unit, int rows_per_wave) {
  const int lane = threadIdx.x & 63, wave = threadIdx.x >> 6;
  const int64_t r0 = ((int64_t)blockIdx.x * 4 + wave) * rows_per_wave;
  float amax = 0.f;
  int64_t unit = amax_out && amax_unit > 0 && r0 < rows ? r0 / amax_unit : 0;
  for (int64_t row = r0; row < r0 + rows_per_wave && row < rows; ++row) {
    const TI* xp = x + row * ldx;
    float v[MAXI];
    float sum = 0.f;
#pragma unroll
// ... 2 lines not shown
      v[i] = idx < C ? ld_act(xp, idx) : 0.f;
      sum += v[i];
    }
    const float mean = wave_sum(sum) / (float)C;
    float sq = 0.f;
#pragma unroll
    for (int i = 0; i < MAXI; ++i) {
      const int idx = lane + 64 * i;
      const float dv = idx < C ? v[i] - mean : 0.f;
      sq += dv * dv;
    }
    const float var = wave_sum(sq) / (float)C;
    const float rstd = 1.0f / sqrtf(var + eps);
    if (amax_out && amax_unit > 0 && row / amax_unit != unit) {
      track_amax(amax_out + unit, amax);
      amax = 0.f;
      unit = row / amax_unit;
    }
    TO* yp = y + row * ldy;
#pragma unroll
    for (int i = 0; i < MAXI; ++i) {
      const int idx = lane + 64 * i;
      if (idx < C) {
        float o = (v[i] - mean) * rstd;
        if (gamma) o = o * gamma[idx] + beta[idx];
        if (gelu) o = gelu_erf(o);
        if (post) o *= post[idx];
        st_act(yp, idx, o);
        amax = fmaxf(amax, fabsf(o));
      } else if (idx < Cpad) {
        st_act(yp, idx, 0.f);
      }
    }
  }
  if (amax_out && r0 < rows) track_amax(amax_out + unit, amax);
}

__global__ __launch_bounds__(256) void amax_kernel(const float* __restrict__ x, int64_t n, float* __restrict__ amax_out) {
  float m = 0.f;
  for (int64_t i = (int64_t)blockIdx.x * 256 + threadIdx.x; i < n; i += (int64_t)gridDim.x * 256) m = fmaxf(m, fabsf(x[i]));
  track_amax(amax_out, m);
}

template <int MAXI>
__global__ __launch_bounds__(256) void row_stats_kernel(const float* __restrict__ x, int64_t ldx, int64_t rows, int C,
                                                        float eps, float* __restrict__ stats) {
  const int lane = threadIdx.x & 63, wave = threadIdx.x >> 6;
  const int64_t row = (int64_t)blockIdx.x * 4 + wave;
  if (row >= rows) return;
  const float* xp = x + row * ldx;
  float v[MAXI];
  float sum = 0.f;
#pragma unroll
  for (int i = 0; i < MAXI; ++i) {
    const int idx = lane + 64 * i;
    v[i] = idx < C ? xp[idx] : 0.f;
    sum += v[i];
  }
  const float mean = wave_sum(sum) / (float)C;
  float sq = 0.f;
#pragma unroll
  for (int i = 0; i < MAXI; ++i) {
    const float dv = lane + 64 * i < C ? v[i] - mean : 0.f;
    sq += dv * dv;
  }
  const float var = wave_sum(sq) / (float)C;
  if (lane == 0) *reinterpret_cast<float2*>(stats + 2 * row) = make_float2(mean, 1.0f / sqrtf(var + eps));
}

__global__ __launch_bounds__(256) void stats_finalize_kernel(const float2* __restrict__ part, int64_t rows, int P, int C,
                                                             float eps, float2* __restrict__ stats) {
  const int64_t r = (int64_t)blockIdx.x * 256 + threadIdx.x;
  if (r >= rows) return;
  double s = 0.0, q = 0.0;
  for (int p = 0; p < P; ++p) {
    const float2 v = part[r * P + p];
    s += (double)v.x;
    q += (double)v.y;
  }
  const double mean = s / C;
  double var = q / C - mean * mean;
  var = var > 0.0 ? var : 0.0;
  stats[r] = make_float2((float)mean, (float)(1.0 / sqrt(var + (double)eps)));
}

__global__ __launch_bounds__(256) void cast_bf16_kernel(const float* __restrict__ x, u16* __restrict__ y,
                                                        int64_t n4) {
  const float4* xs = reinterpret_cast<const float4*>(x);
  ushort4* yd = reinterpret_cast<ushort4*>(y);
  for (int64_t i = (int64_t)blockIdx.x * 256 + threadIdx.x; i < n4; i += (int64_t)gridDim.x * 256) {
    const float4 v = xs[i];
    u16 t[4];
    st_act(t, 0, v.x); st_act(t, 1, v.y); st_act(t, 2, v.z); st_act(t, 3, v.w);
    yd[i] = make_ushort4(t[0], t[1], t[2], t[3]);
  }
}

__global__ __launch_bounds__(1024) void wave_stats_kernel(const float* __restrict__ w, int N,
                                                          float eps, float* __restrict__ stats) {
  __shared__ float red[32];
  const int b = blockIdx.x;
  const float* p = w + (int64_t)b * N;
  const int tid = threadIdx.x, lane = tid & 63, wave = tid >> 6;
  float s = 0.f;
  for (int i = tid; i < N; i += 1024) s += p[i];
  s = wave_sum(s);
  if (lane == 0) red[wave] = s;
  __syncthreads();
  float tot = 0.f;
  for (int i = 0; i < 16; ++i) tot += red[i];
  const float mean = tot / (float)N;
  __syncthreads();
  float q = 0.f;
  for (int i = tid; i < N; i += 1024) {
    const float d = p[i] - mean;
    q += d * d;
  }
  q = wave_sum(q);
  if (lane == 0) red[wave] = q;
  __syncthreads();
  if (tid == 0) {
    float t2 = 0.f;
    for (int i = 0; i < 16; ++i) t2 += red[i];
    stats[2 * b] = mean;
    stats[2 * b + 1] = 1.0f / sqrtf(t2 / (float)N + eps);
  }
}

template <int G, int NV>
__global__ __launch_bounds__(256) void layernorm_v4_kernel(const float* x, int64_t ldx, float* y,
                                                           int64_t ldy, const float* __restrict__ gamma,
                                                           const float* __restrict__ beta, const float* __restrict__ post,
                                                           int64_t rows, int C, int Cpad, float eps, int gelu,
                                                           float* __restrict__ amax_out, int64_t amax_unit, int iters) {
  constexpr int RPW = 64 / G;
  const int lane = threadIdx.x & 63, wave = threadIdx.x >> 6;
  const int sub = lane / G, gl = lane % G;
  const int64_t row0 = ((int64_t)blockIdx.x * 4 + wave) * iters * RPW + sub;
  float4 g4[NV], b4[NV], p4[NV];
#pragma unroll
  for (int k = 0; k < NV; ++k) {
    const int c = 4 * (gl + G * k);
    float gg[4], bb[4], pp[4];
#pragma unroll
    for (int e = 0; e < 4; ++e) {
      const bool in = c + e < C;
      gg[e] = (gamma && in) ? gamma[c + e] : 1.f;
      bb[e] = (beta && gamma && in) ? beta[c + e] : 0.f;
      pp[e] = (post && in) ? post[c + e] : 1.f;
    }
    g4[k] = make_float4(gg[0], gg[1], gg[2], gg[3]);
    b4[k] = make_float4(bb[0], bb[1], bb[2], bb[3]);
    p4[k] = make_float4(pp[0], pp[1], pp[2], pp[3]);
  }
  const float invC = 1.0f / (float)C;
  float seen = -1.f;
  int64_t seen_unit = -1;
  for (int it = 0; it < iters; ++it) {
    const int64_t row = row0 + (int64_t)it * RPW;
    const bool valid = row < rows;
    const int64_t rc = valid ? row : rows - 1;
    const float* xp = x + rc * ldx;
    float4 v[NV];
    float sum = 0.f;
#pragma unroll
    for (int k = 0; k < NV; ++k) {
// ... 65 lines not shown
  if constexpr (std::is_same<TI, float>::value && std::is_same<TO, float>::value) {
    const int needv = Cpad > C ? Cpad : C;
    if (!(needv & 3) && !(ldx & 3) && !(ldy & 3) && needv <= 1024 && !(((uintptr_t)x | (uintptr_t)y) & 15)) {
      int G = 0, NV = 0, best = 1 << 30;
      for (int gcand : {16, 32, 64}) {
        const int nv = (needv + 4 * gcand - 1) / (4 * gcand);
        if (nv <= 4 && nv * 4 * gcand < best) { best = nv * 4 * gcand; G = gcand; NV = nv; }
      }
      if (G) {
        const int rpwv = 64 / G;
        int64_t steps = cdiv64(rows, rpwv);
        int iters = (int)(steps / (2048 * 4));
        iters = iters < 1 ? 1 : (iters > 8 ? 8 : iters);
        const unsigned gridv = (unsigned)cdiv64(cdiv64(steps, iters), 4);
#define DZN_LN4(GV, NVV)                                                                                         \
  hipLaunchKernelGGL((layernorm_v4_kernel<GV, NVV>), dim3(gridv), dim3(256), 0, s, x, ldx, y, ldy, g, b, post, rows, \
                     C, Cpad, eps, gelu, amax, amax_unit, iters)
        if (G == 16 && NV == 1) DZN_LN4(16, 1);
        else if (G == 16 && NV == 2) DZN_LN4(16, 2);
        else if (G == 16 && NV == 3) DZN_LN4(16, 3);
        else if (G == 16 && NV == 4) DZN_LN4(16, 4);
        else if (G == 32 && NV == 3) DZN_LN4(32, 3);
        else if (G == 32 && NV == 4) DZN_LN4(32, 4);
        else if (G == 64 && NV == 3) DZN_LN4(64, 3);
        else if (G == 64 && NV == 4) DZN_LN4(64, 4);
        else G = 0;
#undef DZN_LN4
        if (G) return hipGetLastError() == hipSuccess ? DZN_OK : DZN_E_HIP;
      }
    }
  }
  int rpw = 1;
  if (amax) {
    const int64_t waves = 256 * 4 * 8;
    rpw = (int)(rows / waves);
    rpw = rpw < 1 ? 1 : (rpw > 64 ? 64 : rpw);
  }
  const unsigned grid = (unsigned)cdiv64(cdiv64(rows, rpw), 4);
  const int need = (Cpad > C ? Cpad : C);
#define DZN_LN(MAXI)                                                                               \
  hipLaunchKernelGGL((layernorm_kernel<MAXI, TI, TO>), dim3(grid), dim3(256), 0, s, x, ldx, y, ldy, g, \
                     b, post, rows, C, Cpad, eps, gelu, amax, amax_unit, rpw)
  if (need <= 256) DZN_LN(4);
  else if (need <= 512) DZN_LN(8);
  else if (need <= 1024) DZN_LN(16);
  else DZN_LN(32);
#undef DZN_LN
  return hipGetLastError() == hipSuccess ? DZN_OK : DZN_E_HIP;
}

}

int launch_layernorm_t(const void* x, int x_bf16, int64_t ldx, void* y, int y_bf16, int64_t ldy,
                       const float* g, const float* b, const float* post, int64_t rows, int C, int Cpad,
                       float eps, int gelu, hipStream_t s, float* amax, int64_t amax_unit) {
  ProfScope prof_scope_(s, "layernorm", 0.0, (double)rows * C * 8.0);
  if (rows <= 0) return DZN_OK;
  if (C <= 0 || C > 2048 || Cpad > 2048) return DZN_E_INVALID;
  const float* xf = static_cast<const float*>(x);
  const u16* xh = static_cast<const u16*>(x);
  float* yf = static_cast<float*>(y);
  u16* yh = static_cast<u16*>(y);
  if (!x_bf16 && !y_bf16) return launch_ln_typed(xf, ldx, yf, ldy, g, b, post, rows, C, Cpad, eps, gelu, s, amax, amax_unit);
  if (!x_bf16 && y_bf16) return launch_ln_typed(xf, ldx, yh, ldy, g, b, post, rows, C, Cpad, eps, gelu, s, amax, amax_unit);
  if (x_bf16 && !y_bf16) return launch_ln_typed(xh, ldx, yf, ldy, g, b, post, rows, C, Cpad, eps, gelu, s, amax, amax_unit);
  return launch_ln_typed(xh, ldx, yh, ldy, g, b, post, rows, C, Cpad, eps, gelu, s, amax, amax_unit);
}

int launch_layernorm(const float* x, int64_t ldx, float* y, int64_t ldy, const float* g,
                     const float* b, int64_t rows, int C, int Cpad, float eps, int gelu,
                     hipStream_t s) {
  return launch_layernorm_t(x, 0, ldx, y, 0, ldy, g, b, nullptr, rows, C, Cpad, eps, gelu, s);
}

int launch_stats_finalize(const float* partial, int64_t rows, int P, int C, float eps, float* stats, hipStream_t s) {
  if (rows <= 0) return DZN_OK;
  if (P < 1 || C < 1) return DZN_E_INVALID;
  ProfScope prof_scope_(s, "stats_finalize", 0.0, (double)rows * (P + 1) * 8.0);
  hipLaunchKernelGGL(stats_finalize_kernel, dim3((unsigned)cdiv64(rows, 256)), dim3(256), 0, s,
                     reinterpret_cast<const float2*>(partial), rows, P, C, eps, reinterpret_cast<float2*>(stats));
  return hipGetLastError() == hipSuccess ? DZN_OK : DZN_E_HIP;
}

int launch_amax(const float* x, int64_t n, float* amax, hipStream_t s) {
  if (n <= 0) return DZN_OK;
  int64_t g = cdiv64(n, 256 * 8);
  g = g > 4096 ? 4096 : g;
  hipLaunchKernelGGL(amax_kernel, dim3((unsigned)g), dim3(256), 0, s, x, n, amax);
  return hipGetLastError() == hipSuccess ? DZN_OK : DZN_E_HIP;
}

extern "C" int dzn_op_amax(const float* x, int64_t n, float* amax, void* stream) {
  if (!x || !amax) return DZN_E_INVALID;
  return launch_amax(x, n, amax, reinterpret_cast<hipStream_t>(stream));
}

int launch_row_stats(const float* x, int64_t ldx, int64_t rows, int C, float eps, float* stats, hipStream_t s) {
  if (rows <= 0) return DZN_OK;
  if (C <= 0 || C > 2048) return DZN_E_INVALID;
  const unsigned grid = (unsigned)cdiv64(rows, 4);
  int pid = prof_enabled() ? prof_begin(s, "row_stats", 0.0, (double)rows * C * 4.0) : -1;
#define DZN_RS(MAXI) hipLaunchKernelGGL((row_stats_kernel<MAXI>), dim3(grid), dim3(256), 0, s, x, ldx, rows, C, eps, stats)
  if (C <= 256) DZN_RS(4);
  else if (C <= 512) DZN_RS(8);
  else if (C <= 1024) DZN_RS(16);
  else DZN_RS(32);
#undef DZN_RS
  prof_end(pid, s);
  return hipGetLastError() == hipSuccess ? DZN_OK : DZN_E_HIP;
}

extern "C" int dzn_op_row_stats(const float* x, int64_t ldx, int64_t rows, int32_t C, float eps, float* stats,
                                void* stream) {
  if (!x || !stats) return DZN_E_INVALID;
  return launch_row_stats(x, ldx, rows, C, eps, stats, reinterpret_cast<hipStream_t>(stream));
}

int launch_cast_bf16(const float* x, void* y, int64_t n, hipStream_t s) {
  ProfScope prof_scope_(s, "cast_bf16");
  if (n <= 0) return DZN_OK;
  if (n & 3) return DZN_E_INVALID;
  int64_t g = cdiv64(n / 4, 256);
  g = g > 8192 ? 8192 : g;
  hipLaunchKernelGGL(cast_bf16_kernel, dim3((unsigned)g), dim3(256), 0, s, x, static_cast<u16*>(y), n / 4);
  return hipGetLastError() == hipSuccess ? DZN_OK : DZN_E_HIP;
}

int launch_wave_stats(const float* w, int B, int N, float eps, float* stats, hipStream_t s) {
  ProfScope prof_scope_(s, "wave_stats", 0.0, (double)B * N * 4.0);
  if (B <= 0) return DZN_OK;
  hipLaunchKernelGGL(wave_stats_kernel, dim3(B), dim3(1024), 0, s, w, N, eps, stats);
  return hipGetLastError() == hipSuccess ? DZN_OK : DZN_E_HIP;
}

extern "C" int dzn_op_layernorm(const float* x, int64_t ldx, float* y, int64_t ldy,
                                const float* gamma, const float* beta, int64_t rows, int32_t C,
                                int32_t Cpad, float eps, int32_t gelu, void* stream) {
  if (!x || !y) return DZN_E_INVALID;
  return launch_layernorm(x, ldx, y, ldy, gamma, beta, rows, C, Cpad, eps, gelu,
                          reinterpret_cast<hipStream_t>(stream));
}


namespace {
__global__ __launch_bounds__(256) void fill_u32_kernel(unsigned* __restrict__ p, unsigned v, int64_t n) {
  for (int64_t i = (int64_t)blockIdx.x * 256 + threadIdx.x; i < n; i += (int64_t)gridDim.x * 256) p[i] = v;
}
}

int launch_fill_u32(void* p, unsigned value, int64_t n, hipStream_t st) {
  if (n <= 0) return DZN_OK;
  int64_t g = (n + 255) / 256;
  g = g > 1024 ? 1024 : g;
  hipLaunchKernelGGL(fill_u32_kernel, dim3((unsigned)g), dim3(256), 0, st, static_cast<unsigned*>(p), value, n);
  return hipGetLastError() == hipSuccess ? DZN_OK : DZN_E_HIP;
}
```

diarizen_amd/ops.py:

```python
from __future__ import annotations

import ctypes as C

import torch

from . import _lib
from ._lib import DznGemmDesc, check


def _stream() -> C.c_void_p:
    return C.c_void_p(torch.cuda.current_stream().cuda_stream)


def _p(t):
    return None if t is None else C.c_void_p(t.data_ptr())


def gemm(A, W, *, M=None, N=None, K=None, bias=None, R=None, C_out=None, WS=None, ws_w=0.0,
         ws_init=False, a_rowoff=None, c_rowoff=None, lda=None, kc=0, ldk=0, ldw=None, ldc=None,
         ldws=0, act=0, alpha=1.0, post_relu=False, nz=1, zdiv=1, zs=None, precision=0,
         W16=None, W3=None, a_planes=None, ln_stats=None, ln_colsum=None, W2h=None, col_scale=None,
         a_amax=None, c_amax=None, amax_unit=None, want_row_stats=False, stat_eps=1e-5, mx=False, Wmx=None,
         col_scale_mx=None, kv_col0=None):
    lib = _lib.load()
    assert A.is_cuda and A.dtype in (torch.float32, torch.bfloat16)
    a_bf16 = A.dtype == torch.bfloat16
    if a_bf16 and C_out is None:
        raise ValueError("bf16 A: pass C_out (fp32 or bf16) explicitly")
    if N is None:
        N = W.shape[0]
    if K is None:
        K = W.shape[1]
    if M is None:
        M = A.shape[0]
    if lda is None:
        lda = A.stride(0) if A.dim() == 2 else K
    if ldw is None:
        ldw = W.stride(0) if W is not None else W16.stride(0)
    if C_out is None:
        C_out = torch.empty((M, N), device=A.device, dtype=torch.float32)
    if ldc is None:
        ldc = C_out.stride(0) if C_out.dim() == 2 else N
    if precision in (_lib.DZN_PREC_F32_SPLIT, _lib.DZN_PREC_F32_H2, _lib.DZN_PREC_F16) and W3 is None and K % 32 == 0 and ldw == K and W.is_contiguous():
        W3 = split_weights(W.reshape(-1, K))
    d = DznGemmDesc()
    d.A, d.W, d.W16, d.C = _p(A), _p(W), _p(W16), _p(C_out)
    d.bias, d.R, d.WS = _p(bias), _p(R), _p(WS)
    d.a_rowoff, d.c_rowoff = _p(a_rowoff), _p(c_rowoff)
    d.M, d.N, d.K = M, N, K
    d.lda, d.kc, d.ldk, d.ldw, d.ldc, d.ldws = lda, kc, ldk, ldw, ldc, ldws
    d.act, d.alpha, d.post_relu = act, alpha, int(post_relu)
    d.ws_w, d.ws_init = ws_w, int(ws_init)
    d.nz, d.zdiv = nz, zdiv
    if zs:
        for k, v in zs.items():
            setattr(d, k, v)
    d.precision = precision
    d.a_bf16 = int(a_bf16)
    d.c_bf16 = int(C_out.dtype == torch.bfloat16)
    d.r_bf16 = int(R is not None and R.dtype == torch.bfloat16)
    d.W3 = _p(W3)
    if a_planes is not None:
        d.A = _p(a_planes)
        d.a_split3, d.a_plane = 1, a_planes.stride(0)
    d.ln_stats, d.ln_colsum = _p(ln_stats), _p(ln_colsum)
    if precision in (_lib.DZN_PREC_F32_H2, _lib.DZN_PREC_F16) and W2h is None and K % 32 == 0 and ldw == K and W.is_contiguous():
        W2h, col_scale = split_weights_h2(W.reshape(-1, K))
        if a_amax is None:
            a_amax = amax(A).repeat(max(1, nz // max(zdiv, 1)))
    if mx and Wmx is None:
        assert precision == _lib.DZN_PREC_F16 and K % 32 == 0 and ldw == K and W.is_contiguous()
        Wmx, col_scale_mx = split_weights_mx(W.reshape(-1, K))
    d.W2h, d.col_scale, d.a_amax, d.c_amax = _p(W2h), _p(col_scale), _p(a_amax), _p(c_amax)
    d.Wmx, d.col_scale_mx = _p(Wmx), _p(col_scale_mx)
    d.amax_unit = int(amax_unit) if amax_unit is not None else (max(M, 1) if nz == 1 else 0)
    stats = None
    if want_row_stats:
        part = torch.empty((M, 32, 2), device=A.device, dtype=torch.float32)
        stats = torch.empty((M, 2), device=A.device, dtype=torch.float32)
        d.stat_partial, d.stat_final, d.stat_C, d.stat_eps = _p(part), _p(stats), N, stat_eps
    kvp = kvs = None
    if kv_col0 is not None:
        kvp = torch.zeros((2, M, N - kv_col0), device=A.device, dtype=torch.int16)
        kvs = torch.zeros((M, (N - kv_col0) // 64), device=A.device, dtype=torch.float32)
        d.kv_planes, d.kv_plane_stride, d.kv_scale, d.kv_ld, d.kv_col0 = _p(kvp), kvp.stride(0), _p(kvs), N - kv_col0, kv_col0
    check(lib.dzn_op_gemm(C.byref(d), _stream()), what="dzn_op_gemm")
    if kv_col0 is not None:
        return C_out, kvp, kvs
    return (C_out, stats) if want_row_stats else C_out


def attention_planes(qkv, B, L, h, gate=None, table=None, head_idx=None, Htot=0, scale=0.125):
    lib = _lib.load()
    assert qkv.is_cuda and qkv.dtype == torch.float32 and qkv.shape == (B * L, 3 * h * 64)
    out = torch.empty((B * L, h * 64), device=qkv.device, dtype=torch.float32)
    am = qkv.reshape(B, -1).abs().amax(dim=1).float().contiguous()
    planes = torch.zeros((2, B * L + 64, 2 * h * 64), device=qkv.device, dtype=torch.int16)
    kvs = torch.zeros((B * L + 64, 2 * h), device=qkv.device, dtype=torch.float32)
    check(lib.dzn_op_attention_planes(_p(qkv), _p(out), _p(gate), _p(table), _p(head_idx), B, L, h, Htot, qkv.stride(0),
                                      out.stride(0), scale, _p(am), _p(planes), _p(kvs), _stream()), what="dzn_op_attention_planes")
    return out


def split_weights(W):
    lib = _lib.load()
    assert W.is_cuda and W.dtype == torch.float32 and W.dim() == 2 and W.shape[1] % 32 == 0
    rows, K = W.shape
    out = torch.empty((rows, K // 32, 3, 32), device=W.device, dtype=torch.int16)
    check(lib.dzn_op_split_weights(_p(W), rows, K, W.stride(0), _p(out), _stream()),
          what="dzn_op_split_weights")
    return out


def split_weights_h2(W):
    lib = _lib.load()
    assert W.is_cuda and W.dtype == torch.float32 and W.dim() == 2 and W.shape[1] % 32 == 0
    rows, K = W.shape
    out = torch.empty((rows, K // 32, 2, 32), device=W.device, dtype=torch.int16)
    sc = torch.empty((rows,), device=W.device, dtype=torch.float32)
    check(lib.dzn_op_split_weights_h2(_p(W), rows, K, W.stride(0), _p(out), _p(sc), _stream()),
          what="dzn_op_split_weights_h2")
    return out, sc


def split_weights_mx(W):
    lib = _lib.load()
    assert W.is_cuda and W.dtype == torch.float32 and W.dim() == 2 and W.shape[1] % 32 == 0
    rows, K = W.shape
    out = torch.empty((rows, K // 32, 128), device=W.device, dtype=torch.uint8)
    sc = torch.empty((rows,), device=W.device, dtype=torch.float32)
    check(lib.dzn_op_split_weights_mx(_p(W), rows, K, W.stride(0), _p(out), _p(sc), _stream()),
          what="dzn_op_split_weights_mx")
    return out, sc


def amax(x, out=None):
    lib = _lib.load()
    assert x.is_cuda and x.dtype == torch.float32 and x.is_contiguous()
    if out is None:
        out = torch.zeros((1,), device=x.device, dtype=torch.float32)
    check(lib.dzn_op_amax(_p(x), x.numel(), _p(out), _stream()), what="dzn_op_amax")
    return out


def split_rows(x):
    lib = _lib.load()
    assert x.is_cuda and x.dtype == torch.float32 and x.is_contiguous() and x.shape[1] % 32 == 0
    rows, D = x.shape
    out = torch.empty((3, rows, D), device=x.device, dtype=torch.int16)
    check(lib.dzn_op_split_rows(_p(x), _p(out), out.stride(0), rows, D, _stream()), what="dzn_op_split_rows")
    return out


def conv3x3_c32(img, W3, bias, R=None, relu=False, post_relu=False, out=None, h2_weights=None):
    lib = _lib.load()
    assert img.is_cuda and img.dtype == torch.float32 and img.is_contiguous() and img.shape[-1] == 32
    B, Hp, Wp, _ = img.shape
    if out is None:
        out = torch.zeros_like(img)
    if h2_weights is not None:
        W2h, cs = h2_weights
        am = img.reshape(B, -1).abs().amax(dim=1).float().contiguous()
        check(lib.dzn_op_conv3x3_c32_h2(_p(img), _p(W3), _p(W2h), _p(cs), _p(am), _p(bias), _p(R), _p(out), B, Hp - 2,
# ... 57 lines not shown


class VbxState:

    def __init__(self, X, Phi, gamma0, device: int = -1):
        import numpy as np
        self.np, self.lib = np, _lib.load()
        X = np.ascontiguousarray(X, dtype=np.float64)
        Phi = np.ascontiguousarray(Phi, dtype=np.float64)
        g0 = np.ascontiguousarray(gamma0, dtype=np.float64)
        self.E, self.D = X.shape
        self.K = g0.shape[1]
        assert Phi.shape == (self.D,) and g0.shape[0] == self.E
        self.state = C.c_void_p()
        check(self.lib.dzn_vbx_create(X.ctypes.data_as(C.c_void_p), Phi.ctypes.data_as(C.c_void_p),
                                      g0.ctypes.data_as(C.c_void_p), self.E, self.D, self.K, device,
                                      C.byref(self.state)), what="dzn_vbx_create")

    def stats(self):
        out = self.np.empty((self.K, self.D + 1), dtype=self.np.float64)
        check(self.lib.dzn_vbx_stats(self.state, out.ctypes.data_as(C.c_void_p)), what="dzn_vbx_stats")
        return out

    def estep(self, alpha, ck, lpi, Fa: float) -> float:
        np = self.np
        alpha = np.ascontiguousarray(alpha, dtype=np.float64)
        ck = np.ascontiguousarray(ck, dtype=np.float64)
        lpi = np.ascontiguousarray(lpi, dtype=np.float64)
        assert alpha.shape == (self.K, self.D) and ck.shape == (self.K,) and lpi.shape == (self.K,)
        total = C.c_double(0.0)
        check(self.lib.dzn_vbx_estep(self.state, alpha.ctypes.data_as(C.c_void_p), ck.ctypes.data_as(C.c_void_p),
                                     lpi.ctypes.data_as(C.c_void_p), float(Fa), C.byref(total)), what="dzn_vbx_estep")
        return total.value

    def gamma(self):
        out = self.np.empty((self.E, self.K), dtype=self.np.float64)
        check(self.lib.dzn_vbx_gamma(self.state, out.ctypes.data_as(C.c_void_p)), what="dzn_vbx_gamma")
        return out

    def close(self):
        if self.state:
            self.lib.dzn_vbx_destroy(self.state)
            self.state = C.c_void_p()

    def __del__(self):
        try:
            self.close()
        except Exception:
            pass


def layernorm(x, gamma, beta, C_true=None, eps=1e-5, gelu=False, out=None):
    lib = _lib.load()
    rows, ld = x.shape[0], x.stride(0)
    Cpad = x.shape[1]
    if C_true is None:
        C_true = Cpad
    if out is None:
        out = torch.empty_like(x)
    check(lib.dzn_op_layernorm(_p(x), ld, _p(out), out.stride(0), _p(gamma), _p(beta), rows,
                               C_true, Cpad, eps, int(gelu), _stream()), what="dzn_op_layernorm")
    return out


def row_stats(x, C_true=None, eps=1e-5):
    lib = _lib.load()
    rows = x.shape[0]
    out = torch.empty((rows, 2), device=x.device, dtype=torch.float32)
    check(lib.dzn_op_row_stats(_p(x), x.stride(0), rows, C_true or x.shape[1], eps, _p(out), _stream()),
          what="dzn_op_row_stats")
    return out


def gate_stats(x, gamma, beta, Wg, bg, cst, eps=1e-5):
    lib = _lib.load()
    rows, Htot = x.shape[0], cst.numel()
    gate_ = torch.empty((rows, Htot), device=x.device, dtype=torch.float32)
    stats = torch.empty((rows, 2), device=x.device, dtype=torch.float32)
    check(lib.dzn_op_gate_stats(_p(x), x.stride(0), _p(gamma), _p(beta), _p(Wg), _p(bg), _p(cst), _p(gate_), _p(stats),
                                rows, Htot, eps, _stream()), what="dzn_op_gate_stats")
    return gate_, stats


def gate(y, Wg, bg, cst):
    lib = _lib.load()
    rows = y.shape[0]
    Htot = cst.numel()
    out = torch.empty((rows, Htot), device=y.device, dtype=torch.float32)
    check(lib.dzn_op_gate(_p(y), y.stride(0), _p(Wg), _p(bg), _p(cst), _p(out), rows, Htot,
                          _stream()), what="dzn_op_gate")
    return out


def attention(qkv, B, L, h, *, gate=None, table=None, head_idx=None, Htot=0, scale=0.125,
              precision=0):
    lib = _lib.load()
    out = torch.empty((B * L, h * 64), device=qkv.device, dtype=torch.float32)
    if precision == _lib.DZN_PREC_F32_H2:
        am = qkv.reshape(B, -1).abs().amax(dim=1).float().contiguous()
        check(lib.dzn_op_attention_h2(_p(qkv), _p(out), _p(gate), _p(table), _p(head_idx), B, L, h, Htot,
                                      qkv.stride(0), out.stride(0), scale, _p(am), _stream()), what="dzn_op_attention_h2")
        return out
    check(lib.dzn_op_attention(_p(qkv), _p(out), _p(gate), _p(table), _p(head_idx), B, L, h,
                               Htot, qkv.stride(0), out.stride(0), scale, precision, _stream()),
          what="dzn_op_attention")
    return out
```

include/dzn_ops.h:

```cpp
#ifndef DZN_OPS_H_
#define DZN_OPS_H_

#include <stdint.h>

#ifdef __cplusplus
extern "C" {
#endif

#define DZN_ACT_NONE 0
#define DZN_ACT_GELU 1
#define DZN_ACT_SWISH 2
#define DZN_ACT_RELU 3

typedef struct dzn_gemm_desc {
  const float* A;
  const float* W;
  const void* W16;
  float* C;
  const float* bias;
  const float* R;
  float* WS;
  const int32_t* a_rowoff;
  const int32_t* c_rowoff;
  int32_t M, N, K;
  int64_t lda;
  int32_t kc;
  int64_t ldk;
  int32_t ldw;
  int64_t ldc;
  int64_t ldws;
  int32_t act;
  float alpha;
  int32_t post_relu;
  float ws_w;
  int32_t ws_init;
  int32_t nz, zdiv;
  int64_t a_z0, a_z1, w_z0, w_z1, c_z0, c_z1, b_z0, b_z1;
  int32_t precision;
  double alg_flops;
  int32_t a_bf16;
  int32_t c_bf16;
  int32_t r_bf16;
  const void* W3;
  int32_t a_split3;
  int64_t a_plane;
  const float* ln_stats;
  const float* ln_colsum;
  const void* W2h;
  const float* col_scale;
  const float* a_amax;
  float* c_amax;
  int32_t amax_unit;
  float* stat_partial;
  float* stat_final;
  int32_t stat_C;
  float stat_eps;
  const int32_t* z_count;
  const int32_t* z_list;
  int32_t ln_centered;
  const void* Wmx;
  const float* col_scale_mx;
  int32_t amax_count;
  void* kv_planes;
  int64_t kv_plane_stride;
  float* kv_scale;
  int32_t kv_ld;
  int32_t kv_col0;
} dzn_gemm_desc;

int dzn_op_resblock32_fused(const float* in, float* out, const void* W1, const float* cs1, const float* b1, const void* W2,
                            const float* cs2, const float* b2, const float* amax_in, float l1max1, float bmax1, int32_t B,
                            int32_t Hs, int32_t Ws, void* stream);

int dzn_op_resblock_ws(const float* in, float* out, const void* W1, const float* cs1, const float* b1, const void* W2,
                       const float* cs2, const float* b2, const float* amax_in, float l1max1, float bmax1, int32_t B,
                       int32_t Hs, int32_t Ws, int32_t C, void* stream);

int dzn_op_set_resblock_np(int32_t np);
int dzn_op_set_attention_noskip(int32_t on);

int dzn_op_gemm(const dzn_gemm_desc* d, void* stream);

int dzn_op_split_weights(const float* W, int64_t rows, int32_t K, int64_t ldw, void* W3, void* stream);

int dzn_op_split_weights_h2(const float* W, int64_t rows, int32_t K, int64_t ldw, void* W2h, float* col_scale,
                            void* stream);

int dzn_op_split_weights_mx(const float* W, int64_t rows, int32_t K, int64_t ldw, void* Wmx, float* col_scale,
                            void* stream);
int dzn_checked_status(uint32_t* out4, int32_t reset);

int dzn_op_set_gemm_mx_cfg(const char* cfg);

int dzn_op_set_gemm_cfg(const char* cfg);

int dzn_op_amax(const float* x, int64_t n, float* amax, void* stream);

int dzn_op_split_rows(const float* x, void* planes, int64_t plane_stride, int64_t rows, int32_t D, void* stream);

int dzn_op_conv3x3_c32(const float* in, const void* W3, const float* bias, const float* R, float* out,
                       int32_t B, int32_t Hs, int32_t Ws, int32_t relu, int32_t post_relu, void* stream);

int dzn_op_conv3x3_c32_h2(const float* in, const void* W3, const void* W2h, const float* col_scale, const float* amax_in,
                          const float* bias, const float* R, float* out, int32_t B, int32_t Hs, int32_t Ws,
                          int32_t relu, int32_t post_relu, void* stream);

int dzn_op_layernorm(const float* x, int64_t ldx, float* y, int64_t ldy, const float* gamma,
                     const float* beta, int64_t rows, int32_t C, int32_t Cpad, float eps,
                     int32_t gelu, void* stream);

int dzn_op_row_stats(const float* x, int64_t ldx, int64_t rows, int32_t C, float eps, float* stats, void* stream);

int dzn_op_gate(const float* y, int64_t ldy, const float* Wg, const float* bg, const float* cst,
                float* gate, int64_t rows, int32_t Htot, void* stream);

int dzn_op_gate_stats(const float* x, int64_t ldx, const float* gamma, const float* beta, const float* Wg,
                      const float* bg, const float* cst, float* gate, float* stats, int64_t rows, int32_t Htot,
                      float eps, void* stream);

int dzn_op_attention_h2(const float* qkv, float* out, const float* gate, const float* table, const int32_t* head_idx,
                        int32_t B, int32_t L, int32_t h, int32_t Htot, int32_t ldqkv, int32_t ldo, float scale,
                        const float* amax, void* stream);

int dzn_op_attention_planes(const float* qkv, float* out, const float* gate, const float* table, const int32_t* head_idx,
                            int32_t B, int32_t L, int32_t h, int32_t Htot, int32_t ldqkv, int32_t ldo, float scale,
                            const float* amax, void* planes, float* kvs, void* stream);

int dzn_op_set_attention_qb(int32_t query_blocks_per_wavefront);
int dzn_op_set_attention_prefetch(int32_t on);

int dzn_op_attention(const float* qkv, float* out, const float* gate, const float* table,
                     const int32_t* head_idx, int32_t B, int32_t L, int32_t h,
                     int32_t Htot, int32_t ldqkv, int32_t ldo, float scale,
                     int32_t precision, void* stream);

typedef struct dzn_prof_entry {
  char name[64];
  int64_t launches;
  double ms;
  double flops;
  double bytes;
} dzn_prof_entry;
int dzn_profile_enable(int32_t on);
int dzn_profile_collect(dzn_prof_entry* out, int32_t cap, int32_t* n);
int dzn_profile_reserve(int32_t n_events);

int dzn_op_relpos_bucket(int32_t rel, int32_t num_buckets, int32_t max_distance);

#ifdef __cplusplus
}
#endif
// ... 2 lines not shown
```

Measured before the change: 1743.

## Fuse next layer's LN stats and gate projection into preceding GEMM epilogue

```diff
diff --git a/diarizen_amd/_lib.py b/diarizen_amd/_lib.py
--- a/diarizen_amd/_lib.py
+++ b/diarizen_amd/_lib.py
@@ -93,7 +93,13 @@
         ("amax_count", C.c_int32),
         ("kv_planes", C.c_void_p), ("kv_plane_stride", C.c_int64), ("kv_scale", C.c_void_p), ("kv_ld", C.c_int32),
         ("kv_col0", C.c_int32),
+        ("gate", C.c_void_p), ("gate_gab", C.c_void_p), ("gate_partial", C.c_void_p), ("stat_shift", C.c_void_p),
     ]
+
+
+class DznGateFuse(C.Structure):
+    _fields_ = [("gamma", C.c_void_p), ("beta", C.c_void_p), ("Wg", C.c_void_p), ("bg", C.c_void_p), ("cst", C.c_void_p),
+                ("hc", C.c_void_p), ("gate", C.c_void_p), ("H", C.c_int32)]
 
 
 class DznProfEntry(C.Structure):
@@ -183,6 +189,8 @@
     sig("dzn_op_gate", i32, [vp, i64, vp, vp, vp, vp, i64, i32, vp])
     sig("dzn_op_row_stats", i32, [vp, i64, i64, i32, f32, vp, vp])
     sig("dzn_op_gate_stats", i32, [vp, i64, vp, vp, vp, vp, vp, vp, vp, i64, i32, f32, vp])
+    sig("dzn_op_gate_fold", i32, [vp, vp, vp, vp, i32, vp, vp])
+    sig("dzn_op_gemm_last_fused", i32, [])
     sig("dzn_op_attention_h2", i32, [vp, vp, vp, vp, vp, i32, i32, i32, i32, i32, i32, f32, vp, vp])
     sig("dzn_op_set_attention_qb", i32, [i32])
     sig("dzn_op_set_attention_prefetch", i32, [i32])
@@ -198,7 +206,7 @@
     "dzn_workspace_bytes", "dzn_last_error", "dzn_destroy", "dzn_version", "dzn_linkage_centroid", "dzn_cdist_cosine", "dzn_host_workspace_release",
     "dzn_host_workspace_bytes",
     "dzn_flac_info", "dzn_flac_decode", "dzn_vbx_create", "dzn_vbx_stats", "dzn_vbx_estep", "dzn_vbx_gamma", "dzn_vbx_destroy",
-    "dzn_op_gemm", "dzn_op_split_weights", "dzn_op_split_weights_h2", "dzn_op_split_weights_mx", "dzn_op_set_gemm_mx_cfg", "dzn_checked_status", "dzn_op_set_gemm_cfg", "dzn_op_amax", "dzn_op_conv3x3_c32", "dzn_op_conv3x3_c32_h2", "dzn_op_resblock32_fused", "dzn_op_resblock_ws", "dzn_op_set_resblock_np", "dzn_op_set_attention_noskip", "dzn_op_split_rows", "dzn_op_layernorm", "dzn_op_row_stats", "dzn_op_gate", "dzn_op_gate_stats", "dzn_op_attention", "dzn_op_attention_h2", "dzn_op_attention_planes", "dzn_op_set_attention_qb", "dzn_op_set_attention_prefetch",
+    "dzn_op_gemm", "dzn_op_split_weights", "dzn_op_split_weights_h2", "dzn_op_split_weights_mx", "dzn_op_set_gemm_mx_cfg", "dzn_checked_status", "dzn_op_set_gemm_cfg", "dzn_op_amax", "dzn_op_conv3x3_c32", "dzn_op_conv3x3_c32_h2", "dzn_op_resblock32_fused", "dzn_op_resblock_ws", "dzn_op_set_resblock_np", "dzn_op_set_attention_noskip", "dzn_op_split_rows", "dzn_op_layernorm", "dzn_op_row_stats", "dzn_op_gate", "dzn_op_gate_stats", "dzn_op_gate_fold", "dzn_op_gemm_last_fused", "dzn_op_attention", "dzn_op_attention_h2", "dzn_op_attention_planes", "dzn_op_set_attention_qb", "dzn_op_set_attention_prefetch",
     "dzn_profile_enable", "dzn_profile_collect", "dzn_profile_reserve", "dzn_op_relpos_bucket",
 ]
 
diff --git a/diarizen_amd/csrc/attention.hip b/diarizen_amd/csrc/attention.hip
--- a/diarizen_amd/csrc/attention.hip
+++ b/diarizen_amd/csrc/attention.hip
@@ -311,6 +311,40 @@
   return hipGetLastError() == hipSuccess ? DZN_OK : DZN_E_HIP;
 }
 
+void gate_fold_host(const float* gamma, const float* beta, const float* Wg, const float* bg, int H, float* gab, float* hc) {
+  const int D = 64 * H;
+  double wa[64], wb[64];
+  for (int c = 0; c < 64; ++c) {
+    wa[c] = ((double)Wg[0 * 64 + c] + Wg[1 * 64 + c]) + ((double)Wg[2 * 64 + c] + Wg[3 * 64 + c]);
+    wb[c] = ((double)Wg[4 * 64 + c] + Wg[5 * 64 + c]) + ((double)Wg[6 * 64 + c] + Wg[7 * 64 + c]);
+  }
+  const double ba = ((double)bg[0] + bg[1]) + ((double)bg[2] + bg[3]), bb = ((double)bg[4] + bg[5]) + ((double)bg[6] + bg[7]);
+  for (int h = 0; h < H; ++h) {
+    double sa = 0.0, sb = 0.0, ca = ba, cb = bb;
+    for (int c = 0; c < 64; ++c) {
+      const int n = h * 64 + c;
+      const float fa = (float)((double)gamma[n] * wa[c]), fb = (float)((double)gamma[n] * wb[c]);
+      gab[n] = fa;
+      gab[D + n] = fb;
+      sa += (double)fa;
+      sb += (double)fb;
+      ca += (double)beta[n] * wa[c];
+      cb += (double)beta[n] * wb[c];
+    }
+    hc[4 * h + 0] = (float)sa;
+    hc[4 * h + 1] = (float)sb;
+    hc[4 * h + 2] = (float)ca;
+    hc[4 * h + 3] = (float)cb;
+  }
+}
+
+extern "C" int dzn_op_gate_fold(const float* gamma, const float* beta, const float* Wg, const float* bg, int32_t H, float* gab,
+                                float* hc) {
+  if (!gamma || !beta || !Wg || !bg || !gab || !hc || H < 1 || H > 16) return DZN_E_INVALID;
+  gate_fold_host(gamma, beta, Wg, bg, H, gab, hc);
+  return DZN_OK;
+}
+
 extern "C" int dzn_op_gate_stats(const float* x, int64_t ldx, const float* gamma, const float* beta, const float* Wg,
                                  const float* bg, const float* cst, float* gate, float* stats, int64_t rows,
                                  int32_t Htot, float eps, void* stream) {
diff --git a/diarizen_amd/csrc/common.h b/diarizen_amd/csrc/common.h
--- a/diarizen_amd/csrc/common.h
+++ b/diarizen_amd/csrc/common.h
@@ -112,6 +112,12 @@
 int launch_amax(const float* x, int64_t n, float* amax, hipStream_t s);
 int launch_fill_u32(void* p, unsigned value, int64_t n, hipStream_t st);
 int launch_stats_finalize(const float* partial, int64_t rows, int P, int C, float eps, float* stats, hipStream_t s);
+int launch_gate_finalize(const float* partial, const float* shift, int64_t rows, int H, int C, float eps, const float* hc,
+                         const float* cst, float* stats, float* gate, hipStream_t s);
+enum { DZN_FUSED_GATE = 1, DZN_FUSED_KV_PLANES = 2 };
+void gemm_fused_note(int bit);
+int gemm_last_fused();
+void gate_fold_host(const float* gamma, const float* beta, const float* Wg, const float* bg, int H, float* gab, float* hc);
 int launch_layernorm(const float* x, int64_t ldx, float* y, int64_t ldy, const float* g,
                      const float* b, int64_t rows, int C, int Cpad, float eps, int gelu,
                      hipStream_t s);
diff --git a/diarizen_amd/csrc/engine.cpp b/diarizen_amd/csrc/engine.cpp
--- a/diarizen_amd/csrc/engine.cpp
+++ b/diarizen_amd/csrc/engine.cpp
@@ -58,6 +58,7 @@
   LNp ln1, ln2;
   Lin qkv, out, f1, f2;
   float *Wg = nullptr, *bg = nullptr, *cst = nullptr;
+  float *gab = nullptr, *hc = nullptr;
   int32_t* head_idx = nullptr;
 };
 
@@ -542,6 +543,13 @@
       L.Wg = upload(h, wg.v);
       L.bg = upload(h, bg.v);
       L.cst = upload(h, cs.v);
+      if (h->fold_ln && c.layer_norm_first && D == 64 * h->H && h->H <= 16) {
+        std::vector<float> gab((size_t)2 * D), hc((size_t)4 * h->H);
+        gate_fold_host(need(h, lp + ".layer_norm.weight").v.data(), need(h, lp + ".layer_norm.bias").v.data(), wg.v.data(),
+                       bg.v.data(), h->H, gab.data(), hc.data());
+        L.gab = upload(h, gab);
+        L.hc = upload(h, hc);
+      }
       std::vector<int32_t> hi(c.head_idx[i], c.head_idx[i] + L.h);
       for (int v : hi)
         if (v < 0 || v >= h->H) throw EngineError(DZN_E_INVALID, "head index out of range");
@@ -1175,19 +1183,47 @@
 
   static const bool stats_from_epilogue = getenv("DZN_NO_EPILOGUE_STATS") == nullptr;
   ensure_table(h, L, st);
+  enum { PRE_NONE = 0, PRE_STATS = 1, PRE_GATE = 2 };
+  int pre = PRE_NONE;
+  dzn_gate_fuse greq{};
+  auto carry_next = [&](dzn_gemm_desc& d, int i) -> int {
+    if (!(stats_from_epilogue && fold && c.layer_norm_first && !lp) || i + 1 >= c.n_layers) return PRE_NONE;
+    const EncLayer& Nx = h->layers[i + 1];
+    d.stat_final = h->rstat;
+    d.stat_C = D;
+    d.stat_eps = 1e-5f;
+    if (Nx.attn && Nx.gab) {
+      greq.gamma = Nx.ln1.g; greq.beta = Nx.ln1.b; greq.Wg = Nx.Wg; greq.bg = Nx.bg; greq.cst = Nx.cst;
+      greq.hc = Nx.hc; greq.gate = h->gate; greq.H = h->H;
+      d.gate = &greq;
+      d.gate_gab = Nx.gab;
+      d.gate_partial = h->spart;
+      d.stat_shift = h->rstat;
+      return PRE_GATE;
+    }
+    if (!Nx.attn && Nx.ffn) {
+      d.stat_partial = h->spart;
+      return PRE_STATS;
+    }
+    d.stat_final = nullptr;
+    return PRE_NONE;
+  };
   for (int i = 0; i < c.n_layers; ++i) {
     EncLayer& Ly = h->layers[i];
     const float wl = h->wsum_w[i + 1];
     float* const own = defer ? h->xl + (int64_t)i * ML * D : xr;
-    bool have_stats = false;
+    bool have_stats = pre == PRE_STATS;
+    const bool have_gate = pre == PRE_GATE;
+    pre = PRE_NONE;
     if (Ly.attn) {
       const float* yin = xr;
       bool y16 = false;
       const bool fold1 = fold && c.layer_norm_first;
       if (fold1) {
-        chk(launch_gate_stats(xr, D, Ly.ln1.g, Ly.ln1.b, Ly.Wg, Ly.bg, Ly.cst, h->gate, h->rstat, ML, h->H, 1e-5f,
-                              st),
-            "gate_stats");
+        if (!have_gate)
+          chk(launch_gate_stats(xr, D, Ly.ln1.g, Ly.ln1.b, Ly.Wg, Ly.bg, Ly.cst, h->gate, h->rstat, ML, h->H, 1e-5f,
+                                st),
+              "gate_stats");
       } else if (c.layer_norm_first) {
         ln_t(xr, false, D, h->y, lp, D, Ly.ln1, ML, D, 0, st, nullptr, am(dzn_handle::AM_Y), L);
         yin = h->y;
@@ -1213,7 +1249,8 @@
         d.kv_col0 = hd;
       }
       gemm(d, y16, false, "qkv");
-      if (planes)
+      const bool planes_written = planes && (gemm_last_fused() & DZN_FUSED_KV_PLANES);
+      if (planes_written)
         chk(launch_attention_planes(h->qkv, h->kvp, pstride, h->kvs, 2 * hd, h->ao, h->gate, h->table, Ly.head_idx, B, L, Ly.h, h->H,
                                     3 * hd, hd, 0.125f, st, am(dzn_handle::AM_QKV)),
             "attention");
@@ -1235,6 +1272,8 @@
         o.stat_C = D;
         o.stat_eps = 1e-5f;
         have_stats = true;
+      } else if (!Ly.ffn) {
+        pre = carry_next(o, i);
       }
       gemm(o, lp, false, "out_proj");
       xr = own;
@@ -1263,6 +1302,7 @@
         }
         f2.a_amax = am(dzn_handle::AM_MID);
         f2.c_amax = am(dzn_handle::AM_X);
+        pre = carry_next(f2, i);
         gemm(f2, lp, false, "ffn2");
         xr = own;
       } else if (!defer) {
diff --git a/diarizen_amd/csrc/gemm.hip b/diarizen_amd/csrc/gemm.hip
--- a/diarizen_amd/csrc/gemm.hip
+++ b/diarizen_amd/csrc/gemm.hip
@@ -390,9 +390,39 @@
 
 }
 
+namespace {
+thread_local int t_last_fused = 0;
+
+int launch_gemm_dispatch(dzn_gemm_desc& d, hipStream_t s);
+}
+
+void gemm_fused_note(int bit) { t_last_fused |= bit; }
+int gemm_last_fused() { return t_last_fused; }
+extern "C" int dzn_op_gemm_last_fused(void) { return t_last_fused; }
+
 int launch_gemm(const dzn_gemm_desc& din, hipStream_t s) {
   dzn_gemm_desc d = din;
+  t_last_fused = 0;
   if (d.M <= 0 || d.N <= 0) return DZN_OK;
+  if (!d.gate) {
+    d.gate_partial = nullptr;
+    return launch_gemm_dispatch(d, s);
+  }
+  const dzn_gate_fuse& g = *d.gate;
+  if (!g.gamma || !g.beta || !g.Wg || !g.bg || !g.cst || !g.gate || !d.stat_final || g.H < 1 || g.H > 16 || d.N != 64 * g.H ||
+      d.stat_C != d.N || d.nz > 1 || d.c_rowoff || d.c_bf16)
+    return DZN_E_INVALID;
+  d.stat_partial = nullptr;
+  const bool shape_ok = d.gate_partial && d.gate_gab && g.hc && !(d.ldc & 3) && !(d.ldws & 3) && !d.kv_planes;
+  if (!shape_ok) d.gate_partial = nullptr;
+  const int rc = launch_gemm_dispatch(d, s);
+  if (rc != DZN_OK || (t_last_fused & DZN_FUSED_GATE)) return rc;
+  return launch_gate_stats(d.C, d.ldc > 0 ? d.ldc : d.N, g.gamma, g.beta, g.Wg, g.bg, g.cst, g.gate, d.stat_final, d.M, g.H,
+                           d.stat_eps, s);
+}
+
+namespace {
+int launch_gemm_dispatch(dzn_gemm_desc& d, hipStream_t s) {
   if (d.K <= 0 || (d.K & 7)) return DZN_E_INVALID;
   if (d.kc <= 0) { d.kc = d.K; d.ldk = 0; }
   if (d.kc & 7) return DZN_E_INVALID;
@@ -414,7 +444,7 @@
     const bool ok = d.kv_scale && d.precision == DZN_PREC_F32_H2 && d.W3 && d.W2h && d.col_scale && d.a_amax && !(d.K & 31) &&
                     !(d.kc & 31) && d.ldw == d.K && !d.a_split3 && d.nz == 1 && !d.c_rowoff && d.kv_col0 >= 0 &&
                     d.kv_col0 < d.N && !(d.kv_col0 & 63) && !(d.N & 63) && d.kv_ld == d.N - d.kv_col0 &&
-                    !(d.kv_plane_stride & 3) && d.N > 32 && !getenv("DZN_GEMM_CFG") && !getenv("DZN_NO_H2");
+                    !(d.kv_plane_stride & 3) && d.N > 32;
     if (!ok) return DZN_E_INVALID;
   }
   if (d.ln_centered && !(d.precision == DZN_PREC_F16 && d.W3 && !(d.K & 31) && !(d.kc & 31) && d.ldw == d.K && !d.a_split3))
@@ -424,6 +454,7 @@
     return launch_gemm_split(d, s);
   return launch_prec<false>(d, s);
 }
+}
 
 extern "C" int dzn_op_gemm(const dzn_gemm_desc* d, void* stream) {
   if (!d || !d->A || !d->C) return DZN_E_INVALID;
diff --git a/diarizen_amd/csrc/gemm_epilogue.h b/diarizen_amd/csrc/gemm_epilogue.h
--- a/diarizen_amd/csrc/gemm_epilogue.h
+++ b/diarizen_amd/csrc/gemm_epilogue.h
@@ -143,7 +143,7 @@
   else return v;
 }
 
-template <int BM, int BN, int TM, int TN, int MI, int NI, bool LDSCOLS = false, int RS = 16, int CS = 16>
+template <int BM, int BN, int TM, int TN, int MI, int NI, bool LDSCOLS = false, int RS = 16, int CS = 16, bool GATE = false>
 __device__ __forceinline__ void gemm_epilogue(const dzn_gemm_desc& d, f32x4 (&acc)[MI][NI], int tm, int tn,
                                               int wm, int wn, int lr, int lq, int64_t cz, int64_t bz, int z0 = 0,
                                               const float* row_inv = nullptr, const float* col_scale = nullptr,
@@ -197,6 +197,11 @@
       ln_rs[i] = st.y;
     }
   }
+  float sh[GATE ? MI : 1];
+  if constexpr (GATE) {
+#pragma unroll
+    for (int i = 0; i < MI; ++i) sh[i] = d.stat_shift ? d.stat_shift[2 * (int64_t)mcl[i]] : 0.f;
+  }
   float4 cs4[REGCOLS ? NI : 1], lc4[REGCOLS ? NI : 1], b4[REGCOLS ? NI : 1];
   if constexpr (REGCOLS) {
 #pragma unroll
@@ -228,6 +233,10 @@
       *reinterpret_cast<float4*>(lds_cols + 4 * lane) = c;
       *reinterpret_cast<float4*>(lds_cols + TN + 4 * lane) = l;
       *reinterpret_cast<float4*>(lds_cols + 2 * TN + 4 * lane) = bb;
+      if constexpr (GATE) {
+        *reinterpret_cast<float4*>(lds_cols + 3 * TN + 4 * lane) = *reinterpret_cast<const float4*>(d.gate_gab + n);
+        *reinterpret_cast<float4*>(lds_cols + 4 * TN + 4 * lane) = *reinterpret_cast<const float4*>(d.gate_gab + d.N + n);
+      }
     }
     __builtin_amdgcn_fence(__ATOMIC_RELEASE, "wavefront");
   }
@@ -329,6 +338,33 @@
           }
         }
       }
+      if constexpr (GATE) {
+        static_assert(!GATE || (LDSCOLS && JC % 4 == 0 && RS == 16 && CS == 16 && TN % 64 == 0), "whole head blocks per batch");
+#pragma unroll
+        for (int g4 = 0; g4 < JC / 4; ++g4) {
+          const int jg = jc * JC + g4 * 4;
+          const int nslot = tn * BN + wn * TN + jg * CS;
+          float gs = 0.f, gq = 0.f, ga = 0.f, gb = 0.f;
+#pragma unroll
+          for (int q = 0; q < 4; ++q) {
+            const float* p = lds_cols + 3 * TN + (jg + q) * CS + lq * 4;
+            const float4 a4 = *reinterpret_cast<const float4*>(p), b4g = *reinterpret_cast<const float4*>(p + TN);
+            const float wa_[4] = {a4.x, a4.y, a4.z, a4.w}, wb_[4] = {b4g.x, b4g.y, b4g.z, b4g.w};
+#pragma unroll
+            for (int e = 0; e < 4; ++e) {
+              const float dv = acc[i][jg + q][e] - sh[i];
+              gs += dv;
+              gq = fmaf(dv, dv, gq);
+              ga = fmaf(dv, wa_[e], ga);
+              gb = fmaf(dv, wb_[e], gb);
+            }
+          }
+          gs += __shfl_xor(gs, 16, 64); gq += __shfl_xor(gq, 16, 64); ga += __shfl_xor(ga, 16, 64); gb += __shfl_xor(gb, 16, 64);
+          gs += __shfl_xor(gs, 32, 64); gq += __shfl_xor(gq, 32, 64); ga += __shfl_xor(ga, 32, 64); gb += __shfl_xor(gb, 32, 64);
+          if (lq == 0 && mok[i] && nslot < d.N)
+            reinterpret_cast<float4*>(d.gate_partial)[(int64_t)mcl[i] * (d.N >> 6) + (nslot >> 6)] = make_float4(gs, gq, ga, gb);
+        }
+      }
 #pragma unroll
       for (int jj = 0; jj < JC; ++jj) {
         const int j = jc * JC + jj;
diff --git a/diarizen_amd/csrc/gemm_split.hip b/diarizen_amd/csrc/gemm_split.hip
--- a/diarizen_amd/csrc/gemm_split.hip
+++ b/diarizen_amd/csrc/gemm_split.hip
@@ -20,7 +20,7 @@
   __builtin_amdgcn_s_waitcnt((N & 0xF) | ((N >> 4) << 14) | (0x7 << 4));
 }
 
-template <int BM, int BN, int WGM, int WGN, int S, int NP, int OCC = 1, int ABL = 0, bool RPF = false>
+template <int BM, int BN, int WGM, int WGN, int S, int NP, int OCC = 1, int ABL = 0, bool RPF = false, bool GATE = false>
 __global__ __launch_bounds__(WGM * WGN * 64, OCC) void gemm_split_kernel(const dzn_gemm_desc d, const int ngroups) {
   constexpr int NW = WGM * WGN;
   constexpr int BK = 32;
@@ -298,8 +298,10 @@
         return;
       }
     }
-    gemm_epilogue<BM, BN, TM, TN, MI, NI, true>(d, acc, tm, tn, wm, wn, lr, lq, cz, bz, z0, row_inv, NP <= 2 ? d.col_scale : nullptr,
-                                                reinterpret_cast<float*>(smem) + wave * 3 * TN);
+    static_assert(NW * 5 * TN * 4 <= S * BUF, "column scratch inside the dead stages");
+    gemm_epilogue<BM, BN, TM, TN, MI, NI, true, 16, 16, GATE>(d, acc, tm, tn, wm, wn, lr, lq, cz, bz, z0, row_inv,
+                                                              NP <= 2 ? d.col_scale : nullptr,
+                                                              reinterpret_cast<float*>(smem) + wave * (GATE ? 5 : 3) * TN);
   } else {
     gemm_epilogue<BM, BN, TM, TN, MI, NI>(d, acc, tm, tn, wm, wn, lr, lq, cz, bz, z0, row_inv, NP <= 2 ? d.col_scale : nullptr);
   }
@@ -529,7 +531,10 @@
 }
 
 template <int BM, int BN, int WGM, int WGN, int S, int NP, int OCC = 1, int PRIO = 0>
-int launch_split32_cfg(const dzn_gemm_desc& d, hipStream_t s) {
+int launch_split32_cfg(const dzn_gemm_desc& din, hipStream_t s) {
+  dzn_gemm_desc d = din;
+  d.kv_planes = nullptr;
+  d.gate_partial = nullptr;
   const int tilesM = (d.M + BM - 1) / BM, tilesN = (d.N + BN - 1) / BN;
   const size_t lds = (size_t)S * (BM * 128 + NP * BN * 64);
   auto kern = gemm_split32_kernel<BM, BN, WGM, WGN, S, NP, OCC, PRIO>;
@@ -588,12 +593,22 @@
 }
 
 template <int BM, int BN, int WGM, int WGN, int S, int NP, int OCC = 1, int ABL = 0, bool RPF = false>
-int launch_split_cfg(const dzn_gemm_desc& d, hipStream_t s) {
+int launch_split_cfg(const dzn_gemm_desc& din, hipStream_t s) {
+  dzn_gemm_desc d = din;
   const int tilesM = (d.M + BM - 1) / BM, tilesN = (d.N + BN - 1) / BN;
   const size_t lds = (size_t)S * (BM * 128 + NP * BN * 64);
+  constexpr int TN_ = BN / WGN;
+  constexpr bool HEADS = TN_ % 64 == 0 && ABL == 0;
+  constexpr bool CAN_GATE = HEADS && NP == 2 && !RPF && (BN == 64 || BN == 128) && WGN == 1;
+  if (!HEADS) d.kv_planes = nullptr;
+  if (d.kv_planes) gemm_fused_note(DZN_FUSED_KV_PLANES);
+  if (!CAN_GATE) d.gate_partial = nullptr;
   auto kern = gemm_split_kernel<BM, BN, WGM, WGN, S, NP, OCC, ABL, RPF>;
-  static unsigned long long attr_mask = 0;
-  if (first_use_on_device(attr_mask)) {
+  if constexpr (CAN_GATE) {
+    if (d.gate_partial) kern = gemm_split_kernel<BM, BN, WGM, WGN, S, NP, OCC, ABL, RPF, true>;
+  }
+  static unsigned long long attr_mask[2] = {0, 0};
+  if (first_use_on_device(attr_mask[d.gate_partial ? 1 : 0])) {
     (void)hipFuncSetAttribute(reinterpret_cast<const void*>(kern), hipFuncAttributeMaxDynamicSharedMemorySize,
                               160 * 1024);
   }
@@ -613,6 +628,11 @@
   hipLaunchKernelGGL(kern, grid, dim3(WGM * WGN * 64), lds, s, d, choose_column_groups(d, tilesM, tilesN, BM, NP));
   prof_end(pid, s);
   if (hipGetLastError() != hipSuccess) return DZN_E_HIP;
+  if (d.gate_partial) {
+    gemm_fused_note(DZN_FUSED_GATE);
+    return launch_gate_finalize(d.gate_partial, d.stat_shift, d.M, d.gate->H, d.stat_C, d.stat_eps, d.gate->hc, d.gate->cst,
+                                d.stat_final, d.gate->gate, s);
+  }
   if (d.stat_partial && d.stat_final)
     return launch_stats_finalize(d.stat_partial, d.M, tilesN * WGN, d.stat_C, d.stat_eps, d.stat_final, s);
   return DZN_OK;
diff --git a/diarizen_amd/csrc/norm.hip b/diarizen_amd/csrc/norm.hip
--- a/diarizen_amd/csrc/norm.hip
+++ b/diarizen_amd/csrc/norm.hip
@@ -108,6 +108,35 @@
   double var = q / C - mean * mean;
   var = var > 0.0 ? var : 0.0;
   stats[r] = make_float2((float)mean, (float)(1.0 / sqrt(var + (double)eps)));
+}
+
+__global__ __launch_bounds__(256) void gate_finalize_kernel(const float4* __restrict__ part, const float* shift, int64_t rows,
+                                                            int Hn, int C, float eps, const float4* __restrict__ hc,
+                                                            const float* __restrict__ cst, float* stats, float* __restrict__ gate) {
+  const int hh = threadIdx.x & 15;
+  const int64_t r = (int64_t)blockIdx.x * 16 + (threadIdx.x >> 4);
+  const bool ok = r < rows && hh < Hn;
+  const float4 p = ok ? part[r * Hn + hh] : make_float4(0.f, 0.f, 0.f, 0.f);
+  const double sh = (shift && r < rows) ? (double)shift[2 * r] : 0.0;
+  double s = (double)p.x, q = (double)p.y;
+#pragma unroll
+  for (int o = 1; o < 16; o <<= 1) {
+    s += __shfl_xor(s, o, 16);
+    q += __shfl_xor(q, o, 16);
+  }
+  const double ms = s / C;
+  double var = q / C - ms * ms;
+  var = var > 0.0 ? var : 0.0;
+  const double rstd = 1.0 / sqrt(var + (double)eps);
+  if (ok) {
+    const float4 k = hc[hh];
+    const float ta = (float)(rstd * ((double)p.z - ms * (double)k.x) + (double)k.z);
+    const float tb = (float)(rstd * ((double)p.w - ms * (double)k.y) + (double)k.w);
+    const float ga = 1.0f / (1.0f + expf(-ta));
+    const float gb = 1.0f / (1.0f + expf(-tb));
+    gate[r * Hn + hh] = ga * (gb * cst[hh] - 1.0f) + 2.0f;
+    if (hh == 0) *reinterpret_cast<float2*>(stats + 2 * r) = make_float2((float)(sh + ms), (float)rstd);
+  }
 }
 
 __global__ __launch_bounds__(256) void cast_bf16_kernel(const float* __restrict__ x, u16* __restrict__ y,
@@ -339,6 +368,17 @@
   return hipGetLastError() == hipSuccess ? DZN_OK : DZN_E_HIP;
 }
 
+int launch_gate_finalize(const float* partial, const float* shift, int64_t rows, int H, int C, float eps, const float* hc,
+                         const float* cst, float* stats, float* gate, hipStream_t s) {
+  if (rows <= 0) return DZN_OK;
+  if (H < 1 || H > 16 || C != 64 * H || !partial || !hc || !cst || !stats || !gate) return DZN_E_INVALID;
+  ProfScope prof_scope_(s, "stats_finalize", 0.0, (double)rows * (H * 20.0 + 12.0));
+  hipLaunchKernelGGL(gate_finalize_kernel, dim3((unsigned)cdiv64(rows, 16)), dim3(256), 0, s,
+                     reinterpret_cast<const float4*>(partial), shift, rows, H, C, eps, reinterpret_cast<const float4*>(hc), cst,
+                     stats, gate);
+  return hipGetLastError() == hipSuccess ? DZN_OK : DZN_E_HIP;
+}
+
 int launch_amax(const float* x, int64_t n, float* amax, hipStream_t s) {
   if (n <= 0) return DZN_OK;
   int64_t g = cdiv64(n, 256 * 8);
diff --git a/diarizen_amd/ops.py b/diarizen_amd/ops.py
--- a/diarizen_amd/ops.py
+++ b/diarizen_amd/ops.py
@@ -21,7 +21,7 @@
          ldws=0, act=0, alpha=1.0, post_relu=False, nz=1, zdiv=1, zs=None, precision=0,
          W16=None, W3=None, a_planes=None, ln_stats=None, ln_colsum=None, W2h=None, col_scale=None,
          a_amax=None, c_amax=None, amax_unit=None, want_row_stats=False, stat_eps=1e-5, mx=False, Wmx=None,
-         col_scale_mx=None, kv_col0=None):
+         col_scale_mx=None, kv_col0=None, gate_req=None):
     lib = _lib.load()
     assert A.is_cuda and A.dtype in (torch.float32, torch.bfloat16)
     a_bf16 = A.dtype == torch.bfloat16
@@ -79,6 +79,20 @@
         part = torch.empty((M, 32, 2), device=A.device, dtype=torch.float32)
         stats = torch.empty((M, 2), device=A.device, dtype=torch.float32)
         d.stat_partial, d.stat_final, d.stat_C, d.stat_eps = _p(part), _p(stats), N, stat_eps
+    if gate_req is not None:
+        Hn = gate_req["cst"].numel()
+        gab, hc = gate_fold(gate_req["gamma"], gate_req["beta"], gate_req["Wg"], gate_req["bg"])
+        gpart = torch.empty((M, Hn, 4), device=A.device, dtype=torch.float32)
+        stats = row_stats(R) if R is not None else torch.zeros((M, 2), device=A.device, dtype=torch.float32)
+        gate_out = torch.empty((M, Hn), device=A.device, dtype=torch.float32)
+        gf = _lib.DznGateFuse()
+        gf.gamma, gf.beta, gf.Wg, gf.bg, gf.cst = (_p(gate_req[k]) for k in ("gamma", "beta", "Wg", "bg", "cst"))
+        gf.hc, gf.gate, gf.H = _p(hc), _p(gate_out), Hn
+        d.gate = C.cast(C.pointer(gf), C.c_void_p)
+        d.gate_gab, d.gate_partial, d.stat_shift = _p(gab), _p(gpart), _p(stats)
+        d.stat_final, d.stat_C, d.stat_eps = _p(stats), N, stat_eps
+        check(lib.dzn_op_gemm(C.byref(d), _stream()), what="dzn_op_gemm")
+        return C_out, stats, gate_out, int(lib.dzn_op_gemm_last_fused())
     kvp = kvs = None
     if kv_col0 is not None:
         kvp = torch.zeros((2, M, N - kv_col0), device=A.device, dtype=torch.int16)
@@ -302,6 +316,16 @@
     return gate_, stats
 
 
+def gate_fold(gamma, beta, Wg, bg):
+    lib = _lib.load()
+    Hn = gamma.numel() // 64
+    host = [t.detach().float().cpu().contiguous() for t in (gamma, beta, Wg, bg)]
+    gab = torch.empty((2, 64 * Hn), dtype=torch.float32)
+    hc = torch.empty((Hn, 4), dtype=torch.float32)
+    check(lib.dzn_op_gate_fold(*[_p(t) for t in host], Hn, _p(gab), _p(hc)), what="dzn_op_gate_fold")
+    return gab.to(gamma.device), hc.to(gamma.device)
+
+
 def gate(y, Wg, bg, cst):
     lib = _lib.load()
     rows = y.shape[0]
diff --git a/include/dzn_ops.h b/include/dzn_ops.h
--- a/include/dzn_ops.h
+++ b/include/dzn_ops.h
@@ -66,7 +66,25 @@
   float* kv_scale;
   int32_t kv_ld;
   int32_t kv_col0;
+  const struct dzn_gate_fuse* gate;
+  const float* gate_gab;
+  float* gate_partial;
+  const float* stat_shift;
 } dzn_gemm_desc;
+
+typedef struct dzn_gate_fuse {
+  const float* gamma;
+  const float* beta;
+  const float* Wg;
+  const float* bg;
+  const float* cst;
+  const float* hc;
+  float* gate;
+  int32_t H;
+} dzn_gate_fuse;
+
+int dzn_op_gate_fold(const float* gamma, const float* beta, const float* Wg, const float* bg, int32_t H, float* gab, float* hc);
+int dzn_op_gemm_last_fused(void);
 
 int dzn_op_resblock32_fused(const float* in, float* out, const void* W1, const float* cs1, const float* b1, const void* W2,
                             const float* cs2, const float* b2, const float* amax_in, float l1max1, float bmax1, int32_t B,
```

After: 1755 (median of 6 runs). About the same (+0.7%).
